# saiprasadbarke/robustmvd

Hardware: AMD Instinct MI355X
Metric: depth-maps/sec at 768x1152x4srcx256planes; warp+aggregate HBM GB/s vs roofline (higher is better)
Workload: dtype f32; 1 GPU; mvsnet (Path B) forward 768x1152, 4 source views, 256 planes, batch 1 per step (BASELINE.json configs[2]); the regulariser's two layers with 32 input channels (conv0, conv4): every fp32 operand as two range-scaled fp16 terms on fp16 MFMA, fp32 accumulation (at least as close to a float64 convolution as the fp32 matrix instruction over 1e-42..1e30: tests/test_hip_f16.py), the other nine layers and ; parallelism=1 independent replica(s), frames round-robin, no collectives

## Files before the change

### include/mvd.h

```cpp
#ifndef MVD_H_
#define MVD_H_

#include <stddef.h>

#ifdef __cplusplus
extern "C" {
#endif

#define MVD_VERSION 100
#define MVD_MAX_VIEWS 32

typedef void* mvd_stream_t;

typedef enum {
    MVD_OK = 0,
    MVD_ERR_INVALID_ARG = 1,
    MVD_ERR_WORKSPACE = 2,
    MVD_ERR_LAUNCH = 3,
    MVD_ERR_NO_DEVICE = 4
} mvd_status;

#define MVD_LAYOUT_NCDHW 0
#define MVD_LAYOUT_NDHWC 1
#define MVD_GRID_EXACT 0x100
#define MVD_FEAT_NHWC_BORDER 0x200

#define MVD_LAYOUT_NCHW 0
#define MVD_LAYOUT_NHWC 1
#define MVD_LAYOUT_NHWC_BORDER 2

int mvd_version(void);
const char* mvd_last_error(void);


size_t mvd_sweep_corr_workspace_bytes(int N, int C, int h, int w, int hs, int ws, int V);
int mvd_sweep_corr_f32(const float* feat_key, const float* const* feat_src, const float* K_key,
                       const float* const* K_src, const float* const* T_src2key, const float* invdepths,
                       int invdepth_batched, int N, int C, int h, int w, int hs, int ws, int S, int V,
                       float* const* corr_out, float* const* mask_out, void* workspace, size_t workspace_bytes,
                       mvd_stream_t stream);

#define MVD_INVDEPTH_SHARED 0
#define MVD_INVDEPTH_BATCHED 1
#define MVD_INVDEPTH_PER_PIXEL 2
int mvd_sweep_corr_ex_f32(const float* feat_key, const float* const* feat_src, const float* K_key,
                          const float* const* K_src, const float* const* T_src2key, const float* invdepths,
                          int invdepth_mode, float corr_scale, int N, int C, int h, int w, int hs, int ws, int S, int V,
                          float* const* corr_out, float* const* mask_out, void* workspace, size_t workspace_bytes,
                          mvd_stream_t stream);
int mvd_sweep_corr_nhwc_f32(const float* feat_key, const float* const* feat_src, const float* K_key, const float* const* K_src,
                            const float* const* T_src2key, const float* invdepths, int invdepth_mode, float corr_scale, int N, int C,
                            int h, int w, int hs, int ws, int S, int V, float* const* corr_out, float* const* mask_out,
                            int out_pixel_stride, float* corr_absmax, mvd_stream_t stream);

int mvd_sweep_warp_f32(const float* const* feat_src, const float* K_key, const float* const* K_src,
                       const float* const* T_src2key, const float* invdepths, int invdepth_mode, int normalize_after, int N,
                       int C, int h, int w, int hs, int ws, int S, int V, float* const* warped_out, float* const* mask_out,
                       mvd_stream_t stream);

int mvd_fuse_views_f32(const float* const* corr, const float* const* mask, const float* const* score, int N, int S,
                       int h, int w, int V, float* fused, float* fused_mask, mvd_stream_t stream);
int mvd_fuse_views_nhwc_f32(const float* const* corr, const float* const* mask, const float* const* score, int N, int S, int h,
                            int w, int V, int in_pixel_stride, float* fused, float* fused_mask, int out_pixel_stride,
                            float* fused_absmax, mvd_stream_t stream);


size_t mvd_warp_variance_workspace_bytes(int B, int C, int h, int w, int V);
int mvd_warp_variance_f32(const float* key_feat, const float* const* src_feat, const float* const* src_proj,
                          const float* key_proj_inv, const float* depth_values, int B, int C, int D, int h, int w,
                          int V, float* var_out, int out_layout, void* workspace, size_t workspace_bytes,
                          mvd_stream_t stream);
int mvd_warp_variance_absmax_f32(const float* key_feat, const float* const* src_feat, const float* const* src_proj,
                                 const float* key_proj_inv, const float* depth_values, int B, int C, int D, int h, int w,
                                 int V, float* var_out, float* absmax_out, int out_layout, void* workspace,
                                 size_t workspace_bytes, mvd_stream_t stream);

size_t mvd_warp_variance_f16_workspace_bytes(int B);
int mvd_warp_variance_f16(const void* key_feat, const void* const* src_feat, const float* const* src_proj,
                          const float* key_proj_inv, const float* depth_values, int B, int D, int h, int w, int V,
                          void* var_out, void* workspace, size_t workspace_bytes, mvd_stream_t stream);
int mvd_convert_f32_to_f16(const float* src, void* dst, long long n, mvd_stream_t stream);
int mvd_convert_f16_to_f32(const void* src, float* dst, long long n, mvd_stream_t stream);

int mvd_homo_warp_f32(const float* src_feat, const float* src_proj, const float* key_proj_inv,
                      const float* depth_values, int B, int C, int D, int h, int w, float* warped_out,
                      void* workspace, size_t workspace_bytes, mvd_stream_t stream);

#define MVD_CONV3D_STRIDE1 0
#define MVD_CONV3D_STRIDE2 1
#define MVD_DECONV3D_STRIDE2 2
size_t mvd_conv3d_packed_weight_floats(int Cin, int Cout);
int mvd_pack_conv3d_weights_f32(const float* w, int Cin, int Cout, int mode, float* packed, mvd_stream_t stream);
int mvd_conv3d_bn_relu_f32(const float* x, const float* packed_w, const float* scale, const float* shift,
                           const float* skip, float* y, int B, int Di, int hi, int wi, int Cin, int Cout, int mode,
                           int relu, mvd_stream_t stream);
int mvd_conv3d_bn_relu_absmax_f32(const float* x, const float* packed_w, const float* scale, const float* shift,
                                  const float* skip, float* y, float* absmax_out, int B, int Di, int hi, int wi, int Cin,
                                  int Cout, int mode, int relu, mvd_stream_t stream);

size_t mvd_conv3d_weight_grad_workspace_bytes(int B, int Di, int hi, int wi, int Cin, int Cout, int mode);
int mvd_conv3d_weight_grad_f32(const float* x, const float* gy, float* gw, int B, int Di, int hi, int wi, int Cin, int Cout,
                               int mode, void* workspace, size_t workspace_bytes, mvd_stream_t stream);

size_t mvd_conv3d_f16_packed_weight_bytes(int Cin, int Cout);
int mvd_pack_conv3d_weights_f16(const float* w, int Cin, int Cout, void* packed, mvd_stream_t stream);
int mvd_conv3d_bn_relu_f16in(const void* x, const void* packed_w, const float* scale, const float* shift, float* y, int B,
                             int D, int h, int w, int Cin, int Cout, int relu, mvd_stream_t stream);

size_t mvd_conv3d_split_packed_weight_bytes(int Cin, int Cout);
int mvd_pack_conv3d_weights_split(const float* w, int Cin, int Cout, void* packed, mvd_stream_t stream);
int mvd_conv3d_bn_relu_f32_split(const float* x, const float* x_absmax, const void* packed_w, const float* scale, const float* shift,
                                 float* y, int B, int D, int h, int w, int Cin, int Cout, int relu, mvd_stream_t stream);
int mvd_conv3d_bn_relu_absmax_f32_split(const float* x, const float* x_absmax, const void* packed_w, const float* scale, const float* shift,
                                        float* y, float* y_absmax, int B, int D, int h, int w, int Cin, int Cout, int relu,
                                        mvd_stream_t stream);
size_t mvd_conv3d_igemm_packed_weight_bytes(int Cin, int Cout, int mode);
int mvd_pack_conv3d_weights_igemm(const float* w, int Cin, int Cout, int mode, void* packed, mvd_stream_t stream);
size_t mvd_conv3d_igemm_workspace_bytes(int B, int Di, int Hi, int Wi, int Cin, int Cout, int mode);
int mvd_conv3d_bn_relu_igemm_f32(const float* x, const float* x_absmax, const void* packed_w, const float* scale, const float* shift,
                                 const float* skip, float* y, float* y_absmax, int B, int Di, int Hi, int Wi, int Cin, int Cout, int mode,
                                 int relu, void* workspace, size_t workspace_bytes, mvd_stream_t stream);
#define MVD_CONV2D 0
#define MVD_DECONV2D 1
#define MVD_CONV2D_IMAGE 2
size_t mvd_conv2d_split_packed_weight_bytes(int Cin_pad, int Cout, int KH, int KW, int stride, int mode);
int mvd_pack_conv2d_weights_split(const float* w, int Cin, int Cin_pad, int Cout, int KH, int KW, int stride, int mode, void* packed,
                                  mvd_stream_t stream);
size_t mvd_conv2d_split_workspace_bytes(int B, int Hi, int Wi, int Cin_pad, int Cout, int KH, int KW, int stride, int mode);
int mvd_conv2d_split_f32(const float* x, const float* x_absmax, const void* packed_w, const float* bias, float* y, float* y_absmax, int B,
                         int Hi, int Wi, int Cin_pad, int x_pixel_stride, int Cout, int y_pixel_stride, long long y_row_stride,
                         long long y_image_stride, long long y_channel_stride, int KH, int KW, int stride, int mode, int act, float slope,
                         void* workspace, size_t workspace_bytes, mvd_stream_t stream);
int mvd_upsample2x_nhwc_f32(const float* x, float* y, float* y_absmax, int B, int C, int h, int w, int y_pixel_stride, mvd_stream_t stream);
int mvd_absmax_f32(const float* x, long long n, float* absmax, mvd_stream_t stream);

size_t mvd_conv2d_packed_weight_floats(int Cin, int Cout, int ksize);
int mvd_pack_conv2d_weights_f32(const float* w, int Cin, int Cout, int ksize, float* packed, mvd_stream_t stream);
int mvd_conv2d_bn_relu_f32(const float* x, int in_layout, const float* packed_w, const float* scale, const float* shift,
                           float* y, int out_layout, int B, int hi, int wi, int Cin, int Cout, int ksize, int stride,
                           int relu, mvd_stream_t stream);
int mvd_conv2d_bn_relu_absmax_f32(const float* x, int in_layout, const float* packed_w, const float* scale, const float* shift,
                                  float* y, float* y_absmax, int out_layout, int B, int hi, int wi, int Cin, int Cout, int ksize,
                                  int stride, int relu, mvd_stream_t stream);

size_t mvd_conv2d_head_tile_count(int B, int H, int W);
int mvd_conv2d_head_f32(const float* image, const float* w0, const float* scale0, const float* shift0, const float* w1,
                        const float* scale1, const float* shift1, float* y, float* tile_absmax, int B, int H, int W,
                        mvd_stream_t stream);

int mvd_softmax_regress_f32(const float* cost, const float* depth_values, int B, int D, int h, int w,
                            float* depth_out, float* conf_out, mvd_stream_t stream);

int mvd_softmax_regress_stats_f32(const float* cost, const float* depth_values, int B, int D, int h, int w,
                                  float* depth_out, float* conf_out, float* stats_out, mvd_stream_t stream);
int mvd_softmax_regress_backward_f32(const float* cost, const float* depth_values, const float* depth, const float* stats,
                                     const float* g_depth, int B, int D, int h, int w, float* g_cost, mvd_stream_t stream);

int mvd_stream_fill_f32(float* dst, long long n, float value, mvd_stream_t stream);

int mvd_arm_kernel_timing(void* start_event, void* stop_event);

int mvd_bias_leaky_relu_f32(float* x, const float* bias, int N, int C, long long HW, float slope, mvd_stream_t stream);

#define MVD_REDUCE_VARIANCE 0
#define MVD_REDUCE_VARIANCE_KEYSQ 1
#define MVD_REDUCE_GROUPCORR 2
size_t mvd_sweep_reduce_workspace_bytes(int B, int C, int h, int w, int V);
int mvd_sweep_reduce_f32(const float* key_feat, const float* const* src_feat, const float* const* M, const float* depth,
                         int depth_per_pixel, float pix_offset, float scale_x, float scale_y, float bias, int mode, int groups,
                         int B, int C, int D, int h, int w, int V, float* const* out, void* workspace, size_t workspace_bytes,
                         mvd_stream_t stream);

int mvd_sweep_reduce_nhwc_f32(const float* key_feat, const float* const* src_feat, const float* const* M, const float* depth,
                              int depth_per_pixel, float pix_offset, float scale_x, float scale_y, float bias, int mode, int B, int C,
                              int D, int h, int w, int V, float* out, mvd_stream_t stream);

int mvd_softmax_regress_pp_f32(const float* cost, const float* depth_hypos, int B, int D, int h, int w, float* depth_out,
                               float* conf_out, mvd_stream_t stream);

int mvd_sweep_groupcorr_nhwc_f32(const float* key_feat, const float* const* src_feat, const float* const* M, const float* depth,
                                 int depth_per_pixel, float pix_offset, float scale_x, float scale_y, float bias, float grid_clamp,
                                 int groups, int B, int C, int D, int h, int w, int V, float* const* out, mvd_stream_t stream);

int mvd_soft_argmin_f32(const float* score, const float* depth_start, int start_per_pixel, const float* depth_interval, float window,
                        int B, int D, int h, int w, float* depth_out, float* entropy_out, float* prob_map_out, mvd_stream_t stream);

int mvd_vis_fuse_f32(const float* const* x, const float* const* u, int B, int D, int h, int w, int C, int V, float* out,
                     mvd_stream_t stream);


size_t mvd_warp_variance_backward_workspace_bytes(int B);
int mvd_warp_variance_backward_f32(const float* key_feat, const float* const* src_feat, const float* const* src_proj,
                                   const float* key_proj_inv, const float* depth_values, const float* grad_var, int B, int C,
                                   int D, int h, int w, int V, float* grad_key, float* const* grad_src, void* workspace,
                                   size_t workspace_bytes, mvd_stream_t stream);

#define MVD_K3_GATHER_RADIUS 3
size_t mvd_warp_variance_backward_gather_workspace_bytes(int B, int C, int D, int h, int w, int V);
int mvd_warp_variance_backward_gather_f32(const float* key_feat, const float* const* src_feat, const float* const* src_proj,
                                          const float* key_proj_inv, const float* depth_values, const float* grad_var, int B, int C,
                                          int D, int h, int w, int V, float* grad_key, float* const* grad_src, int* fallback_count,
                                          void* workspace, size_t workspace_bytes, mvd_stream_t stream);

int mvd_sweep_corr_backward_f32(const float* feat_key, const float* const* feat_src, const float* K_key,
                                const float* const* K_src, const float* const* T_src2key, const float* invdepths,
                                int invdepth_mode, float corr_scale, const float* const* grad_corr, int N, int C, int h, int w,
                                int hs, int ws, int S, int V, float* grad_key, float* const* grad_src, mvd_stream_t stream);

int mvd_sweep_warp_backward_f32(const float* K_key, const float* const* K_src, const float* const* T_src2key, const float* invdepths,
                                int invdepth_mode, const float* const* grad_warped, int N, int C, int h, int w, int hs, int ws, int S,
                                int V, float* const* grad_src, mvd_stream_t stream);

size_t mvd_sweep_reduce_backward_workspace_bytes(int B, int C, int h, int w, int V);
int mvd_sweep_reduce_backward_f32(const float* key_feat, const float* const* src_feat, const float* const* M, const float* depth,
                                  int depth_per_pixel, float pix_offset, float scale_x, float scale_y, float bias, int mode,
                                  int groups, const float* const* grad_out, int B, int C, int D, int h, int w, int V, float* grad_key,
                                  float* const* grad_src, void* workspace, size_t workspace_bytes, mvd_stream_t stream);

int mvd_fuse_views_backward_f32(const float* const* corr, const float* const* mask, const float* const* score,
                                const float* grad_fused, int N, int S, int h, int w, int V, float* const* grad_corr,
                                float* const* grad_score, mvd_stream_t stream);

int mvd_resize_order1_f32(const float* src, float* dst, long long planes, int hi, int wi, int ho, int wo,
                          mvd_stream_t stream);

int mvd_dispnet_head_f32(const float* x, float* pred, float* ent, int N, long long HW, mvd_stream_t stream);

#define MVD_ALIGN_NONE 0
#define MVD_ALIGN_MEDIAN 1
#define MVD_ALIGN_LSQ 2
size_t mvd_depth_eval_workspace_bytes(int H, int W);

int mvd_depth_align_stats_f32(const float* gt, const float* pred, const float* uncertainty, const int* row, const int* col, int H,
                              int W, int h, int w, int mode, int sparse_pred, float* params, double* sums, void* workspace,
                              size_t workspace_bytes, mvd_stream_t stream);

int mvd_depth_score_f32(const float* gt, const float* pred, const float* uncertainty, const int* row, const int* col, int H, int W,
                        int h, int w, int mode, int sparse_pred, int clip, float clip_lo, float clip_hi, float thresh,
                        float thresh_plus_one, const float* params, void* result, float* pred_out, float* invdepth_out,
                        float* rel_ae_out, float* uncertainty_out, void* workspace, size_t workspace_bytes, mvd_stream_t stream);

int mvd_rank_keys_f32(const float* u, const float* u_min, const float* gt, const float* pred_aligned, int sparse_pred, long long n,
                      float* keys, mvd_stream_t stream);

int mvd_ranked_step_sums_f64(const float* ranked, long long n, const long long* count, double* step_sums, void* workspace,
                             size_t workspace_bytes, mvd_stream_t stream);

int mvd_geo_consistency_f32(const float* key_depth, const float* const* src_depth, const float* matrices, const float* uncertainty,
                            int V, int H, int W, float max_reproj_error, float max_rel_depth_diff, int min_consistent_views,
                            float max_uncertainty, unsigned* view_bits, float* fused, unsigned char* mask,
                            unsigned char* num_consistent, mvd_stream_t stream);

size_t mvd_compact_points_workspace_bytes(int H, int W);
int mvd_compact_points_f32(const unsigned char* mask, const float* depth, const float* image, const float* backproject, int H, int W,
                           float* xyz, float* rgb, long long* count, void* workspace, size_t workspace_bytes, mvd_stream_t stream);

#define MVD_CLOUD_MAX_THRESHOLDS 8
int mvd_cloud_cell_keys_f32(const float* points, long long n, double origin_x, double origin_y, double origin_z, double inv,
                            long long* keys, mvd_stream_t stream);

int mvd_cloud_grid_build_f32(const float* points, const long long* perm, long long n, float* records, mvd_stream_t stream);

int mvd_cloud_nearest_f32(const float* query_records, long long n, const float* target_records, const long long* target_keys,
                          long long m, double origin_x, double origin_y, double origin_z, double inv, float max_dist, float* dist,
                          int* index, mvd_stream_t stream);

size_t mvd_cloud_scores_workspace_bytes(long long n);
int mvd_cloud_scores_f32(const float* dist, const int* index, const float* points, long long n, const float* thresholds, int T,
                         void* result, void* workspace, size_t workspace_bytes, mvd_stream_t stream);

size_t mvd_voxel_reduce_workspace_bytes(long long n);
int mvd_voxel_reduce_f32(const long long* keys, const long long* perm, const float* points, const float* colors, long long n,
                         float* xyz, float* rgb, int* counts, long long* num_voxels, void* workspace, size_t workspace_bytes,
                         mvd_stream_t stream);

int mvd_nchw_to_nhwc_f32(const float* src, float* dst, int N, int C, long long HW, mvd_stream_t stream);
int mvd_nhwc_to_nchw_f32(const float* src, float* dst, int N, int C, long long HW, mvd_stream_t stream);

#ifdef __cplusplus
}
#endif
#endif
```

### robustmvd_amd/_lib.py

```python
import ctypes
import os

import torch

_HERE = os.path.dirname(os.path.abspath(__file__))
LIB_PATH = os.path.join(_HERE, "lib", "libmvd_hip.so")
EXP_LIB_PATH = os.path.join(_HERE, "lib_exp", "libmvd_hip_exp.so")

MVD_MAX_VIEWS = 32
LAYOUT_NCDHW = 0
LAYOUT_NDHWC = 1
GRID_EXACT = 0x100
FEAT_NHWC_BORDER = 0x200
CONV3D_STRIDE1 = 0
CONV2D, DECONV2D, CONV2D_IMAGE = 0, 1, 2
CONV3D_STRIDE2 = 1
DECONV3D_STRIDE2 = 2
LAYOUT_NCHW = 0
LAYOUT_NHWC = 1
LAYOUT_NHWC_BORDER = 2
INVDEPTH_SHARED, INVDEPTH_BATCHED, INVDEPTH_PER_PIXEL = 0, 1, 2
REDUCE_VARIANCE = 0
REDUCE_VARIANCE_KEYSQ = 1
REDUCE_GROUPCORR = 2
ALIGN_NONE, ALIGN_MEDIAN, ALIGN_LSQ = 0, 1, 2
K3_GATHER_RADIUS = 3

_c_float_p = ctypes.c_void_p
_pp = ctypes.POINTER(ctypes.c_void_p)
_i = ctypes.c_int
_sz = ctypes.c_size_t

SIGNATURES = {
    "mvd_version": (_i, []),
    "mvd_last_error": (ctypes.c_char_p, []),
    "mvd_sweep_corr_workspace_bytes": (_sz, [_i] * 7),
    "mvd_sweep_corr_f32": (_i, [_c_float_p, _pp, _c_float_p, _pp, _pp, _c_float_p, _i] + [_i] * 8
                           + [_pp, _pp, ctypes.c_void_p, _sz, ctypes.c_void_p]),
    "mvd_sweep_corr_ex_f32": (_i, [_c_float_p, _pp, _c_float_p, _pp, _pp, _c_float_p, _i, ctypes.c_float] + [_i] * 8
                              + [_pp, _pp, ctypes.c_void_p, _sz, ctypes.c_void_p]),
    "mvd_sweep_corr_nhwc_f32": (_i, [_c_float_p, _pp, _c_float_p, _pp, _pp, _c_float_p, _i, ctypes.c_float] + [_i] * 8
                                + [_pp, _pp, _i, _c_float_p, ctypes.c_void_p]),
    "mvd_fuse_views_nhwc_f32": (_i, [_pp, _pp, _pp] + [_i] * 6 + [_c_float_p, _c_float_p, _i, _c_float_p, ctypes.c_void_p]),
    "mvd_upsample2x_nhwc_f32": (_i, [_c_float_p, _c_float_p, _c_float_p] + [_i] * 5 + [ctypes.c_void_p]),
    "mvd_sweep_warp_f32": (_i, [_pp, _c_float_p, _pp, _pp, _c_float_p] + [_i] * 10 + [_pp, _pp, ctypes.c_void_p]),
    "mvd_fuse_views_f32": (_i, [_pp, _pp, _pp, _i, _i, _i, _i, _i, _c_float_p, _c_float_p, ctypes.c_void_p]),
    "mvd_warp_variance_workspace_bytes": (_sz, [_i] * 5),
    "mvd_warp_variance_f32": (_i, [_c_float_p, _pp, _pp, _c_float_p, _c_float_p] + [_i] * 6
                              + [_c_float_p, _i, ctypes.c_void_p, _sz, ctypes.c_void_p]),
    "mvd_warp_variance_absmax_f32": (_i, [_c_float_p, _pp, _pp, _c_float_p, _c_float_p] + [_i] * 6
                                     + [_c_float_p, _c_float_p, _i, ctypes.c_void_p, _sz, ctypes.c_void_p]),
    "mvd_absmax_f32": (_i, [_c_float_p, ctypes.c_longlong, _c_float_p, ctypes.c_void_p]),
    "mvd_warp_variance_f16_workspace_bytes": (_sz, [_i]),
    "mvd_warp_variance_f16": (_i, [ctypes.c_void_p, _pp, _pp, _c_float_p, _c_float_p] + [_i] * 5
                              + [ctypes.c_void_p, ctypes.c_void_p, _sz, ctypes.c_void_p]),
    "mvd_convert_f32_to_f16": (_i, [_c_float_p, ctypes.c_void_p, ctypes.c_longlong, ctypes.c_void_p]),
    "mvd_convert_f16_to_f32": (_i, [ctypes.c_void_p, _c_float_p, ctypes.c_longlong, ctypes.c_void_p]),
    "mvd_homo_warp_f32": (_i, [_c_float_p] * 4 + [_i] * 5 + [_c_float_p, ctypes.c_void_p, _sz, ctypes.c_void_p]),
    "mvd_conv3d_packed_weight_floats": (_sz, [_i, _i]),
    "mvd_pack_conv3d_weights_f32": (_i, [_c_float_p, _i, _i, _i, _c_float_p, ctypes.c_void_p]),
    "mvd_conv3d_bn_relu_f32": (_i, [_c_float_p] * 6 + [_i] * 8 + [ctypes.c_void_p]),
    "mvd_conv3d_bn_relu_absmax_f32": (_i, [_c_float_p] * 7 + [_i] * 8 + [ctypes.c_void_p]),
    "mvd_conv3d_weight_grad_workspace_bytes": (_sz, [_i] * 7),
    "mvd_conv3d_weight_grad_f32": (_i, [_c_float_p] * 3 + [_i] * 7 + [ctypes.c_void_p, _sz, ctypes.c_void_p]),
    "mvd_conv3d_f16_packed_weight_bytes": (_sz, [_i, _i]),
    "mvd_pack_conv3d_weights_f16": (_i, [_c_float_p, _i, _i, ctypes.c_void_p, ctypes.c_void_p]),
    "mvd_conv3d_bn_relu_f16in": (_i, [ctypes.c_void_p, ctypes.c_void_p, _c_float_p, _c_float_p, _c_float_p] + [_i] * 7
                                 + [ctypes.c_void_p]),
    "mvd_conv3d_split_packed_weight_bytes": (_sz, [_i, _i]),
    "mvd_conv3d_bn_relu_absmax_f32_split": (_i, [_c_float_p, _c_float_p, ctypes.c_void_p, _c_float_p, _c_float_p, _c_float_p, _c_float_p]
                                            + [_i] * 7 + [ctypes.c_void_p]),
    "mvd_conv3d_igemm_packed_weight_bytes": (_sz, [_i] * 3),
    "mvd_pack_conv3d_weights_igemm": (_i, [_c_float_p, _i, _i, _i, ctypes.c_void_p, ctypes.c_void_p]),
    "mvd_conv3d_igemm_workspace_bytes": (_sz, [_i] * 7),
    "mvd_conv3d_bn_relu_igemm_f32": (_i, [_c_float_p, _c_float_p, ctypes.c_void_p] + [_c_float_p] * 5 + [_i] * 8
                                     + [ctypes.c_void_p, ctypes.c_size_t, ctypes.c_void_p]),
    "mvd_conv2d_split_packed_weight_bytes": (_sz, [_i] * 6),
    "mvd_pack_conv2d_weights_split": (_i, [_c_float_p] + [_i] * 7 + [ctypes.c_void_p, ctypes.c_void_p]),
    "mvd_conv2d_split_workspace_bytes": (_sz, [_i] * 9),
    "mvd_conv2d_split_f32": (_i, [_c_float_p, _c_float_p, ctypes.c_void_p, _c_float_p, _c_float_p, _c_float_p] + [_i] * 7
                             + [ctypes.c_longlong] * 3 + [_i] * 5 + [ctypes.c_float, ctypes.c_void_p, ctypes.c_size_t, ctypes.c_void_p]),
    "mvd_pack_conv3d_weights_split": (_i, [_c_float_p, _i, _i, ctypes.c_void_p, ctypes.c_void_p]),
    "mvd_conv3d_bn_relu_f32_split": (_i, [_c_float_p, _c_float_p, ctypes.c_void_p, _c_float_p, _c_float_p, _c_float_p] + [_i] * 7
                                     + [ctypes.c_void_p]),
    "mvd_conv2d_packed_weight_floats": (_sz, [_i, _i, _i]),
    "mvd_pack_conv2d_weights_f32": (_i, [_c_float_p, _i, _i, _i, _c_float_p, ctypes.c_void_p]),
    "mvd_conv2d_bn_relu_f32": (_i, [_c_float_p, _i, _c_float_p, _c_float_p, _c_float_p, _c_float_p, _i] + [_i] * 8
                               + [ctypes.c_void_p]),
    "mvd_conv2d_head_tile_count": (_sz, [_i] * 3),
    "mvd_conv2d_head_f32": (_i, [_c_float_p] * 9 + [_i] * 3 + [ctypes.c_void_p]),
    "mvd_conv2d_bn_relu_absmax_f32": (_i, [_c_float_p, _i, _c_float_p, _c_float_p, _c_float_p, _c_float_p, _c_float_p, _i] + [_i] * 8
                                      + [ctypes.c_void_p]),
    "mvd_softmax_regress_f32": (_i, [_c_float_p, _c_float_p, _i, _i, _i, _i, _c_float_p, _c_float_p, ctypes.c_void_p]),
    "mvd_softmax_regress_stats_f32": (_i, [_c_float_p, _c_float_p, _i, _i, _i, _i, _c_float_p, _c_float_p, _c_float_p,
                                           ctypes.c_void_p]),
    "mvd_softmax_regress_backward_f32": (_i, [_c_float_p] * 5 + [_i] * 4 + [_c_float_p, ctypes.c_void_p]),
    "mvd_bias_leaky_relu_f32": (_i, [_c_float_p, _c_float_p, _i, _i, ctypes.c_longlong, ctypes.c_float, ctypes.c_void_p]),
    "mvd_dispnet_head_f32": (_i, [_c_float_p, _c_float_p, _c_float_p, _i, ctypes.c_longlong, ctypes.c_void_p]),
    "mvd_arm_kernel_timing": (_i, [ctypes.c_void_p, ctypes.c_void_p]),
    "mvd_stream_fill_f32": (_i, [_c_float_p, ctypes.c_longlong, ctypes.c_float, ctypes.c_void_p]),
    "mvd_warp_variance_backward_workspace_bytes": (_sz, [_i]),
    "mvd_warp_variance_backward_f32": (_i, [_c_float_p, _pp, _pp, _c_float_p, _c_float_p, _c_float_p] + [_i] * 6
                                       + [_c_float_p, _pp, ctypes.c_void_p, _sz, ctypes.c_void_p]),
    "mvd_warp_variance_backward_gather_workspace_bytes": (_sz, [_i] * 6),
    "mvd_warp_variance_backward_gather_f32": (_i, [_c_float_p, _pp, _pp, _c_float_p, _c_float_p, _c_float_p] + [_i] * 6
                                              + [_c_float_p, _pp, ctypes.c_void_p, ctypes.c_void_p, _sz, ctypes.c_void_p]),
    "mvd_sweep_corr_backward_f32": (_i, [_c_float_p, _pp, _c_float_p, _pp, _pp, _c_float_p, _i, ctypes.c_float, _pp] + [_i] * 8
                                    + [_c_float_p, _pp, ctypes.c_void_p]),
    "mvd_fuse_views_backward_f32": (_i, [_pp, _pp, _pp, _c_float_p] + [_i] * 5 + [_pp, _pp, ctypes.c_void_p]),
    "mvd_sweep_reduce_workspace_bytes": (_sz, [_i] * 5),
    "mvd_sweep_reduce_f32": (_i, [_c_float_p, _pp, _pp, _c_float_p, _i] + [ctypes.c_float] * 4 + [_i] * 8
                             + [_pp, ctypes.c_void_p, _sz, ctypes.c_void_p]),
    "mvd_sweep_reduce_nhwc_f32": (_i, [_c_float_p, _pp, _pp, _c_float_p, _i] + [ctypes.c_float] * 4 + [_i] * 7
                                  + [_c_float_p, ctypes.c_void_p]),
    "mvd_softmax_regress_pp_f32": (_i, [_c_float_p, _c_float_p, _i, _i, _i, _i, _c_float_p, _c_float_p, ctypes.c_void_p]),
    "mvd_sweep_groupcorr_nhwc_f32": (_i, [_c_float_p, _pp, _pp, _c_float_p, _i] + [ctypes.c_float] * 5 + [_i] * 7 + [_pp, ctypes.c_void_p]),
    "mvd_soft_argmin_f32": (_i, [_c_float_p, _c_float_p, _i, _c_float_p, ctypes.c_float] + [_i] * 4 + [_c_float_p] * 3 + [ctypes.c_void_p]),
    "mvd_vis_fuse_f32": (_i, [_pp, _pp] + [_i] * 6 + [_c_float_p, ctypes.c_void_p]),
    "mvd_sweep_reduce_backward_workspace_bytes": (_sz, [_i] * 5),
    "mvd_sweep_reduce_backward_f32": (_i, [_c_float_p, _pp, _pp, _c_float_p, _i] + [ctypes.c_float] * 4 + [_i, _i, _pp] + [_i] * 6
                                      + [_c_float_p, _pp, ctypes.c_void_p, _sz, ctypes.c_void_p]),
    "mvd_sweep_warp_backward_f32": (_i, [_c_float_p, _pp, _pp, _c_float_p, _i, _pp] + [_i] * 8 + [_pp, ctypes.c_void_p]),
    "mvd_resize_order1_f32": (_i, [_c_float_p, _c_float_p, ctypes.c_longlong, _i, _i, _i, _i, ctypes.c_void_p]),
    "mvd_nchw_to_nhwc_f32": (_i, [_c_float_p, _c_float_p, _i, _i, ctypes.c_longlong, ctypes.c_void_p]),
    "mvd_nhwc_to_nchw_f32": (_i, [_c_float_p, _c_float_p, _i, _i, ctypes.c_longlong, ctypes.c_void_p]),
    "mvd_depth_eval_workspace_bytes": (_sz, [_i, _i]),
    "mvd_depth_align_stats_f32": (_i, [_c_float_p] * 3 + [ctypes.c_void_p] * 2 + [_i] * 6 + [_c_float_p, ctypes.c_void_p,
                                                                                            ctypes.c_void_p, _sz, ctypes.c_void_p]),
    "mvd_depth_score_f32": (_i, [_c_float_p] * 3 + [ctypes.c_void_p] * 2 + [_i] * 7 + [ctypes.c_float] * 4
                            + [_c_float_p, ctypes.c_void_p] + [_c_float_p] * 4 + [ctypes.c_void_p, _sz, ctypes.c_void_p]),
    "mvd_rank_keys_f32": (_i, [_c_float_p] * 4 + [_i, ctypes.c_longlong, _c_float_p, ctypes.c_void_p]),
    "mvd_ranked_step_sums_f64": (_i, [_c_float_p, ctypes.c_longlong, ctypes.c_void_p, ctypes.c_void_p, ctypes.c_void_p, _sz,
                                      ctypes.c_void_p]),
    "mvd_geo_consistency_f32": (_i, [_c_float_p, _pp, _c_float_p, _c_float_p, _i, _i, _i, ctypes.c_float, ctypes.c_float, _i,
                                     ctypes.c_float] + [ctypes.c_void_p] * 5),
    "mvd_compact_points_workspace_bytes": (_sz, [_i, _i]),
    "mvd_compact_points_f32": (_i, [ctypes.c_void_p] + [_c_float_p] * 3 + [_i, _i, _c_float_p, _c_float_p, ctypes.c_void_p,
                                                                          ctypes.c_void_p, _sz, ctypes.c_void_p]),
    "mvd_cloud_cell_keys_f32": (_i, [_c_float_p, ctypes.c_longlong] + [ctypes.c_double] * 4 + [ctypes.c_void_p] * 2),
    "mvd_cloud_grid_build_f32": (_i, [_c_float_p, ctypes.c_void_p, ctypes.c_longlong, _c_float_p, ctypes.c_void_p]),
    "mvd_cloud_nearest_f32": (_i, [_c_float_p, ctypes.c_longlong, _c_float_p, ctypes.c_void_p, ctypes.c_longlong]
                              + [ctypes.c_double] * 4 + [ctypes.c_float, _c_float_p, ctypes.c_void_p, ctypes.c_void_p]),
    "mvd_cloud_scores_workspace_bytes": (_sz, [ctypes.c_longlong]),
    "mvd_cloud_scores_f32": (_i, [_c_float_p, ctypes.c_void_p, _c_float_p, ctypes.c_longlong, _c_float_p, _i, ctypes.c_void_p,
                                  ctypes.c_void_p, _sz, ctypes.c_void_p]),
    "mvd_voxel_reduce_workspace_bytes": (_sz, [ctypes.c_longlong]),
    "mvd_voxel_reduce_f32": (_i, [ctypes.c_void_p] * 2 + [_c_float_p] * 2 + [ctypes.c_longlong, _c_float_p, _c_float_p]
                             + [ctypes.c_void_p] * 3 + [_sz, ctypes.c_void_p]),
}
MVD_CLOUD_MAX_THRESHOLDS = 8

PRODUCT_ONLY = ("mvd_sweep_reduce_backward_workspace_bytes", "mvd_sweep_reduce_backward_f32")

_lib = None
_override = None


def _bind(path, skip=()):
    lib = ctypes.CDLL(path)
    for name, (res, args) in SIGNATURES.items():
        if name in skip:
            continue
        fn = getattr(lib, name)
        fn.restype = res
        fn.argtypes = args
    return lib


def load():
    global _lib
    if _override is not None:
        return _override
    if _lib is not None:
        return _lib
    if not os.path.exists(LIB_PATH):
        raise RuntimeError(
            f"{LIB_PATH} not found: the HIP engine is not built. Run `python -c 'import __graft_entry__ as g; "
            "g.build()'` or `make -C robustmvd_amd/csrc`. There is no CPU fallback for this path.")
    _lib = _bind(LIB_PATH)
    return _lib


class use_experiments_library:

    def __init__(self, path=None):
        self.path = path or EXP_LIB_PATH

    def __enter__(self):
        global _override
        if not os.path.exists(self.path):
            raise RuntimeError(f"{self.path} not found: run `make -C robustmvd_amd/csrc exp`")
        self._prev = _override
        _override = _bind(self.path, skip=PRODUCT_ONLY)
        return _override

    def __exit__(self, *exc):
        global _override
        _override = self._prev
        return False


def check(rc, what):
    if rc != 0:
        msg = load().mvd_last_error().decode(errors="replace")
        raise RuntimeError(f"{what} failed (status {rc}): {msg}")


def stream_of(t):
    return ctypes.c_void_p(torch.cuda.current_stream(t.device).cuda_stream)


def raw_stream(device):
    return torch._C._cuda_getCurrentRawStream(device.index)


def ptr(t):
    return ctypes.c_void_p(t.data_ptr()) if t is not None else ctypes.c_void_p(0)


def ptr_array(tensors):
    arr = (ctypes.c_void_p * len(tensors))(*[t.data_ptr() for t in tensors])
    return ctypes.cast(arr, _pp), arr


def as_dtype(dtype, convert, t, name, shape=None, device=None):
    if not isinstance(t, torch.Tensor):
        raise ValueError(f"{name}: expected a torch.Tensor, got {type(t).__name__}")
    if not t.is_cuda:
        raise ValueError(f"{name}: tensor is on {t.device}; the HIP engine needs a cuda (ROCm) device tensor")
    if device is not None and t.device != device:
        raise ValueError(f"{name}: on {t.device}, expected {device}")
    if t.dtype != dtype:
        if not convert:
            raise ValueError(f"{name}: dtype {t.dtype}, expected {dtype}")
        t = t.to(dtype)
    if shape is not None and t.shape != tuple(shape):
        raise ValueError(f"{name}: shape {tuple(t.shape)}, expected {tuple(shape)}")
    return t.contiguous()


def as_f32(t, name, shape=None, device=None):
    return as_dtype(torch.float32, True, t, name, shape, device)


def as_f16(t, name, shape=None, device=None):
    return as_dtype(torch.float16, False, t, name, shape, device)
```

### robustmvd_amd/blocks.py

```python
import numpy as np
import torch
import torch.nn as nn
import torch.nn.functional as F

from . import _lib as L
from . import ops
from .utils import to_torch

homo_warp = ops.homo_warp


def compute_sampling_invdepths(min_depth, max_depth, num_samples, sampling_type="linear_invdepth"):
    def col(v):
        if isinstance(v, (float, int, np.floating)):
            v = torch.tensor([float(v)])
        return to_torch(v).float()[..., None]

    lo, hi = col(min_depth), col(max_depth)
    steps = torch.arange(0, num_samples, dtype=lo.dtype, device=lo.device)[None]
    if sampling_type == "linear_invdepth":
        return 1 / hi + steps * (1 / lo - 1 / hi) / (num_samples - 1)
    if sampling_type == "linear_depth":
        return (1 / (lo + steps * (hi - lo) / (num_samples - 1))).flip(1)
    raise ValueError(f"sampling_type {sampling_type!r}")


class PlanesweepCorrelation(nn.Module):

    def __init__(self, warp_only=False, normalize="dim", differentiable=False):
        super().__init__()
        self.warp_only = bool(warp_only)
        self.differentiable = bool(differentiable)
        allowed = ("dim", "before", "after", True, False) if warp_only else ("dim", "before", True, False)
        if normalize not in allowed:
            raise ValueError(f"normalize={normalize!r}: expected one of {allowed}")
        self.normalize = normalize
        self._invdepth_cache = {}

    def warm(self, num_sampling_points, min_depth, max_depth, sampling_type, device):
        ckey = (num_sampling_points, float(min_depth), float(max_depth), sampling_type, str(device))
        if ckey not in self._invdepth_cache:
            self._invdepth_cache[ckey] = compute_sampling_invdepths(min_depth, max_depth, num_sampling_points,
                                                                    sampling_type).to(device)
        return self._invdepth_cache[ckey]

    def forward(self, feat_key, intrinsics_key, feat_sources, source_to_key_transforms, intrinsics_sources=None,
                num_sampling_points=None, min_depth=None, max_depth=None, sampling_invdepths=None,
                sampling_type="linear_invdepth"):
        args = (feat_key, intrinsics_key, feat_sources, source_to_key_transforms, intrinsics_sources, num_sampling_points,
                min_depth, max_depth, sampling_invdepths, sampling_type)
        if self.warp_only:
            if ops.needs_grad(feat_sources):
                if not self.differentiable:
                    raise ValueError("PlanesweepCorrelation(warp_only=True): a source feature map requires grad; construct the "
                                     "block with differentiable=True for the engine's backward, or detach the features")
                return self._forward(ops.sweep_warp_autograd, *args)
            with torch.no_grad():
                return self._forward(ops.sweep_warp, *args)
        if ops.needs_grad(feat_key, feat_sources):
            return self._forward(ops.sweep_corr_autograd, *args)
        with torch.no_grad():
            return self._forward(ops.sweep_corr, *args)

    def _forward(self, sweep, feat_key, intrinsics_key, feat_sources, source_to_key_transforms, intrinsics_sources,
                 num_sampling_points, min_depth, max_depth, sampling_invdepths, sampling_type):
        if intrinsics_sources is None:
            intrinsics_sources = [intrinsics_key] * len(feat_sources)
        if not (len(feat_sources) == len(source_to_key_transforms) == len(intrinsics_sources)):
            raise ValueError("feat_sources, source_to_key_transforms and intrinsics_sources differ in length")
        if min_depth is not None and max_depth is not None:
            if sampling_invdepths is not None or num_sampling_points is None or sampling_type is None:
                raise ValueError("give either (num_sampling_points, min_depth, max_depth) or sampling_invdepths")
            scalars = all(isinstance(v, (float, int, np.floating)) for v in (min_depth, max_depth))
            ckey = (num_sampling_points, float(min_depth), float(max_depth), sampling_type, str(feat_key.device)) if scalars else None
            if ckey is not None and ckey in self._invdepth_cache:
                sampling_invdepths = self._invdepth_cache[ckey]
            else:
                sampling_invdepths = compute_sampling_invdepths(min_depth, max_depth, num_sampling_points, sampling_type)
                if ckey is not None:
                    sampling_invdepths = self._invdepth_cache[ckey] = sampling_invdepths.to(feat_key.device)
        elif num_sampling_points is not None or min_depth is not None or max_depth is not None or sampling_invdepths is None:
            raise ValueError("give either (num_sampling_points, min_depth, max_depth) or sampling_invdepths")
        inv = sampling_invdepths.to(feat_key.device)
        if inv.dim() < 2 or inv.dim() > 4:
            raise ValueError("sampling_invdepths must be (N, S), (N, S, H) or (N, S, H, W)")
        while inv.dim() < 4:
            inv = inv.unsqueeze(-1)
        inv_out = inv
        if inv.shape[2] == 1 and inv.shape[3] == 1:
            inv = inv.reshape(inv.shape[0], inv.shape[1])
        else:
            inv = inv.expand(feat_key.shape[0], inv.shape[1], feat_key.shape[2], feat_key.shape[3]).contiguous()
        if self.warp_only:
            srcs = list(feat_sources)
            if self.normalize == "before":
                srcs = [f / (torch.linalg.norm(f, dim=1, keepdim=True) + 1e-9) for f in srcs]
            after = self.normalize is True or self.normalize == "after"
            warped, masks = [None] * len(srcs), [None] * len(srcs)
            groups = {}
            for i, f in enumerate(srcs):
                groups.setdefault(tuple(f.shape[-2:]), []).append(i)
            for idxs in groups.values():
                wv, mv = sweep([srcs[i] for i in idxs], intrinsics_key, [intrinsics_sources[i] for i in idxs],
                                        [source_to_key_transforms[i] for i in idxs], inv, feat_key.shape[-2:], after)
                for i, wi, mi in zip(idxs, wv, mv):
                    warped[i], masks[i] = wi, mi
            return warped, masks, inv_out
        corr_scale = None
        if self.normalize != "dim":
            corr_scale = 1.0
            if self.normalize:
                nrm = lambda x: x / (torch.linalg.norm(x, dim=1, keepdim=True) + 1e-9)
                feat_key, feat_sources = nrm(feat_key), [nrm(f) for f in feat_sources]
        corrs = [None] * len(feat_sources)
        masks = [None] * len(feat_sources)
        groups = {}
        for i, f in enumerate(feat_sources):
            groups.setdefault(tuple(f.shape[-2:]), []).append(i)
        for idxs in groups.values():
            c, m = sweep(feat_key, [feat_sources[i] for i in idxs], intrinsics_key,
                         [intrinsics_sources[i] for i in idxs], [source_to_key_transforms[i] for i in idxs], inv, corr_scale)
            for i, ci, mi in zip(idxs, c, m):
                corrs[i], masks[i] = ci, mi
        return corrs, masks, inv_out


class LearnedFusion(nn.Module):
    def __init__(self):
        super().__init__()
        self.corr_to_view_weight = nn.Sequential(
            nn.Conv2d(256, 128, kernel_size=3, stride=1, padding=1, bias=True),
            nn.ReLU(inplace=True),
            nn.Conv2d(128, 1, kernel_size=1, stride=1, padding=0, bias=True),
        )

    def forward(self, corrs, masks):
        if len(corrs) == 1:
            return corrs[0], masks[0]
        n = corrs[0].shape[0]
        scores = self.corr_to_view_weight(torch.cat(list(corrs), 0))
        scores = list(torch.split(scores, n, 0))
        if ops.needs_grad(corrs, scores):
            return ops.fuse_views_autograd(corrs, masks, scores)
        return ops.fuse_views(corrs, masks, scores)


def depth_regression(p, depth_values):
    return torch.sum(p * depth_values.view(*depth_values.shape, 1, 1), 1)


class ConvBnReLU(nn.Module):
    def __init__(self, cin, cout, kernel_size=3, stride=1, pad=1):
        super().__init__()
        self.conv = nn.Conv2d(cin, cout, kernel_size, stride=stride, padding=pad, bias=False)
        self.bn = nn.BatchNorm2d(cout)

    def forward(self, x):
        return F.relu(self.bn(self.conv(x)), inplace=True)


def fold_bn(bn):
    scale = bn.weight / torch.sqrt(bn.running_var + bn.eps)
    return scale.detach().contiguous(), (bn.bias - bn.running_mean * scale).detach().contiguous()


class FeatureNetWeights:
    __slots__ = ("layers", "split", "head")

    def __init__(self):
        self.layers, self.split, self.head = [], [], ()

    def __getitem__(self, i):
        return self.layers[i]


class FeatureNet(nn.Module):

    SPEC = [(3, 8, 3, 1, 1), (8, 8, 3, 1, 1), (8, 16, 5, 2, 2), (16, 16, 3, 1, 1), (16, 16, 3, 1, 1),
            (16, 32, 5, 2, 2), (32, 32, 3, 1, 1)]

    def __init__(self, split_layers=True):
        super().__init__()
        self.inplanes = 32
        self.split_layers = bool(split_layers)
        self.fused_head = True
        for i, s in enumerate(self.SPEC):
            setattr(self, f"conv{i}", ConvBnReLU(*s))
        self.feature = nn.Conv2d(32, 32, 3, 1, 1)
        self._packed = None
        self._packed_key = None

    def _prepare(self):
        key = tuple((p.data_ptr(), p._version) for p in list(self.parameters()) + list(self.buffers()))
        if self._packed is not None and self._packed_key == key:
            return self._packed
        if self.training:
            raise RuntimeError("FeatureNet HIP path folds BatchNorm running statistics: call .eval() first")
        pk = FeatureNetWeights()
        for i, (cin, cout, k, stride, _) in enumerate(self.SPEC):
            m = getattr(self, f"conv{i}")
            w, _, _, _ = ops.pack_conv2d_weights(m.conv.weight.detach())
            pk.layers.append((w, cin, cout, k, stride, *fold_bn(m.bn), True))
        w, _, _, _ = ops.pack_conv2d_weights(self.feature.weight.detach())
        pk.layers.append((w, 32, 32, 3, 1, torch.ones(32, device=w.device), self.feature.bias.detach().contiguous(), False))
        if self.split_layers:
            for i in range(2, 8):
                conv = getattr(self, f"conv{i}").conv if i < 7 else self.feature
                _, _, _, _, stride, scale, shift, relu = pk.layers[i]
                pk.split.append((ops.pack_conv2d_weights_split(conv.weight.detach() * scale.view(-1, 1, 1, 1), shift, stride=stride), relu))
            for i in range(2):
                _, _, _, _, _, scale, shift, _ = pk.layers[i]
                pk.head += (getattr(self, f"conv{i}").conv.weight.detach().permute(2, 3, 1, 0).contiguous(), scale, shift)
        self._packed, self._packed_key = pk, key
        return pk

    @ops.inference_only
    def forward_layout(self, x, out_layout, return_absmax=False):
        pk = self._prepare()
        if not self.split_layers:
            for i, (w, cin, cout, k, stride, scale, shift, relu) in enumerate(pk.layers):
                x = ops.conv2d_bn_relu(x, w, cin, cout, k, stride, scale, shift, relu=relu,
                                       out_layout=out_layout if i == len(pk.layers) - 1 else L.LAYOUT_NHWC)
            return (x, ops.absmax(x)) if return_absmax else x
        slots = torch.zeros(8, dtype=torch.float32, device=x.device)
        if self.fused_head:
            x, a_in = ops.conv2d_head(x, *pk.head, return_absmax=True)
        else:
            for w, cin, cout, k, stride, scale, shift, relu in pk.layers[:2]:
                x = ops.conv2d_bn_relu(x, w, cin, cout, k, stride, scale, shift, relu=relu)
            a_in = ops.absmax(x)
        for j, (wts, relu) in enumerate(pk.split):
            last = j == len(pk.split) - 1
            if not last:
                x = ops.conv2d_split(x, a_in, wts, act=2 if relu else 0, out_absmax=slots[j:j + 1])
                a_in = slots[j:j + 1]
            elif out_layout == L.LAYOUT_NCHW:
                x = ops.conv2d_split(x, a_in, wts, act=0, planar_out=True)
                if return_absmax:
                    slots[7:8] = ops.absmax(x)
            elif out_layout == L.LAYOUT_NHWC_BORDER:
                B, h, w_, _ = x.shape
                buf = torch.zeros((B, h + 3, w_ + 3, wts.cout), dtype=torch.float32, device=x.device)
                ops.conv2d_split(x, a_in, wts, act=0, out=buf[:, 1:h + 1, 1:w_ + 1, :], out_absmax=slots[7:8])
                x = buf
            else:
                x = ops.conv2d_split(x, a_in, wts, act=0, out_absmax=slots[7:8])
        if return_absmax:
            return x, slots[7:8]
        return x

    def forward(self, x):
        return self.forward_layout(x, L.LAYOUT_NCHW)

    def forward_autograd(self, x):
        x = self.conv1(self.conv0(x))
        x = self.conv4(self.conv3(self.conv2(x)))
        return self.feature(self.conv6(self.conv5(x)))


class ConvBnReLU3D(nn.Module):
    def __init__(self, cin, cout, kernel_size=3, stride=1, pad=1):
        super().__init__()
        self.conv = nn.Conv3d(cin, cout, kernel_size, stride=stride, padding=pad, bias=False)
        self.bn = nn.BatchNorm3d(cout)

    def forward(self, x):
        return F.relu(self.bn(self.conv(x)), inplace=True)


def _deconv_block(cin, cout):
    return nn.Sequential(nn.ConvTranspose3d(cin, cout, kernel_size=3, padding=1, output_padding=1, stride=2, bias=False),
                         nn.BatchNorm3d(cout), nn.ReLU(inplace=True))


class CostRegNet(nn.Module):

    LAYERS = [("conv0", 32, 8, 1), ("conv1", 8, 16, 2), ("conv2", 16, 16, 1), ("conv3", 16, 32, 2), ("conv4", 32, 32, 1),
              ("conv5", 32, 64, 2), ("conv6", 64, 64, 1)]
    UPS = [("conv7", 64, 32), ("conv9", 32, 16), ("conv11", 16, 8)]

    def __init__(self, conv0_split=True):
        super().__init__()
        self.conv0_split = bool(conv0_split)
        for name, cin, cout, stride in self.LAYERS:
            setattr(self, name, ConvBnReLU3D(cin, cout, stride=stride))
        for name, cin, cout in self.UPS:
            setattr(self, name, _deconv_block(cin, cout))
        self.prob = nn.Conv3d(8, 1, 3, stride=1, padding=1)
        self._packed = None
        self._packed_key = None

    def _prepare(self):
        key = tuple((p.data_ptr(), p._version) for p in list(self.parameters()) + list(self.buffers()))
        if self._packed is not None and self._packed_key == key:
            return self._packed
        if self.training:
            raise RuntimeError("CostRegNet HIP path folds BatchNorm running statistics: call .eval() first")
        pk = {}
        for name, cin, cout, stride in self.LAYERS:
            m = getattr(self, name)
            mode = L.CONV3D_STRIDE1 if stride == 1 else L.CONV3D_STRIDE2
            w, _, _ = ops.pack_conv3d_weights(m.conv.weight.detach(), mode)
            pk[name] = (w, cin, cout, *fold_bn(m.bn), mode)
        for name, cin, cout in self.UPS:
            m = getattr(self, name)
            w, _, _ = ops.pack_conv3d_weights(m[0].weight.detach(), L.DECONV3D_STRIDE2)
            pk[name] = (w, cin, cout, *fold_bn(m[1]), L.DECONV3D_STRIDE2)
        w, _, _ = ops.pack_conv3d_weights(self.prob.weight.detach(), L.CONV3D_STRIDE1)
        pk["prob"] = (w, 8, 1, torch.ones(1, device=w.device), self.prob.bias.detach().contiguous(), L.CONV3D_STRIDE1)
        pk["conv0_f16"] = ops.pack_conv3d_weights_f16(self.conv0.conv.weight.detach())
        if self.conv0_split:
            pk["conv0_split"] = ops.pack_conv3d_weights_split(self.conv0.conv.weight.detach())
            sc0, sh0 = pk["conv0"][3], pk["conv0"][4]
            pk["conv0_bound"] = ((self.conv0.conv.weight.detach().abs().sum(dim=(1, 2, 3, 4)) * sc0.abs()).contiguous(), sh0.abs().contiguous())
            for name, _, _, stride in self.LAYERS:
                if name != "conv0":
                    pk[name + "_igemm"] = ops.pack_conv3d_weights_igemm(getattr(self, name).conv.weight.detach(),
                                                                        L.CONV3D_STRIDE1 if stride == 1 else L.CONV3D_STRIDE2)
        self._packed, self._packed_key = pk, key
        return pk

    @ops.inference_only
    def forward_channels_last(self, x, x_absmax=None):
        if x.shape[1] % 8 or x.shape[2] % 8 or x.shape[3] % 8:
            raise ValueError(f"CostRegNet needs D,h,w divisible by 8, got {tuple(x.shape[1:4])}")
        pk = self._prepare()

        def layer(name, t, relu=True, skip=None):
            w, cin, cout, scale, shift, mode = pk[name]
            return ops.conv3d_bn_relu(t, w, cin, cout, scale, shift, mode, relu=relu, skip=skip)

        if x.dtype == torch.float16:
            _, _, _, scale0, shift0, _ = pk["conv0"]
            conv0 = ops.conv3d_bn_relu_f16in(x, pk["conv0_f16"], scale0, shift0, relu=True)
            a0 = None
        elif self.conv0_split:
            _, _, _, scale0, shift0, _ = pk["conv0"]
            if x_absmax is None:
                x_absmax = ops.absmax(x)
            conv0 = ops.conv3d_bn_relu_split(x, pk["conv0_split"], scale0, shift0, relu=True, x_absmax=x_absmax)
            gain0, off0 = pk["conv0_bound"]
            a0 = (gain0 * x_absmax + off0).amax().reshape(1)
        else:
            conv0 = layer("conv0", x)
        if self.conv0_split:
            slots = torch.zeros(8, dtype=torch.float32, device=x.device)
            nslot = [0]

            def ig(name, t, a, want_absmax=True):
                _, cin, cout, sc, sh, mode = pk[name]
                out_a = None
                if want_absmax:
                    out_a = slots[nslot[0]:nslot[0] + 1]
                    nslot[0] += 1
                return ops.conv3d_bn_relu_igemm(t, a, pk[name + "_igemm"], cin, cout, sc, sh, mode, relu=True, return_absmax=want_absmax,
                                                out_absmax=out_a)

            if a0 is None:
                a0 = ops.absmax(conv0)
            t, a = ig("conv1", conv0, a0)
            conv2, a = ig("conv2", t, a)
            t, a = ig("conv3", conv2, a)
            conv4, a = ig("conv4", t, a)
            t, a = ig("conv5", conv4, a)
            y = ig("conv6", t, a, want_absmax=False)
        else:
            conv2 = layer("conv2", layer("conv1", conv0))
            conv4 = layer("conv4", layer("conv3", conv2))
            y = layer("conv6", layer("conv5", conv4))
        y = layer("conv7", y, skip=conv4)
        del conv4
        y = layer("conv9", y, skip=conv2)
        del conv2
        y = layer("conv11", y, skip=conv0)
        del conv0
        return layer("prob", y, relu=False).squeeze(-1)

    @ops.inference_only
    def forward(self, x):
        return self.forward_channels_last(ops.to_channels_last_3d(x)).unsqueeze(1)

    def forward_autograd(self, x):
        conv0 = self.conv0(x)
        conv2 = self.conv2(self.conv1(conv0))
        conv4 = self.conv4(self.conv3(conv2))
        x = self.conv6(self.conv5(conv4))
        x = conv4 + self.conv7(x)
        x = conv2 + self.conv9(x)
        x = conv0 + self.conv11(x)
        return self.prob(x)

    def forward_autograd_engine(self, x):
        if x.dim() != 5 or x.shape[1] % 8 or x.shape[2] % 8 or x.shape[3] % 8:
            raise ValueError(f"CostRegNet needs (B,D,h,w,32) with D,h,w divisible by 8, got {tuple(x.shape)}")

        def layer(name, t):
            m = getattr(self, name)
            stride = m.conv.stride[0]
            y = ops.conv3d_autograd(t, m.conv.weight, L.CONV3D_STRIDE1 if stride == 1 else L.CONV3D_STRIDE2)
            return F.relu(_batch_norm_channels_last(m.bn, y), inplace=True)

        def up(name, t):
            m = getattr(self, name)
            y = ops.conv3d_autograd(t, m[0].weight, L.DECONV3D_STRIDE2)
            return F.relu(_batch_norm_channels_last(m[1], y), inplace=True)

        conv0 = layer("conv0", x)
        conv2 = layer("conv2", layer("conv1", conv0))
        conv4 = layer("conv4", layer("conv3", conv2))
        x = layer("conv6", layer("conv5", conv4))
        x = conv4 + up("conv7", x)
        x = conv2 + up("conv9", x)
        x = conv0 + up("conv11", x)
        return (ops.conv3d_autograd(x, self.prob.weight, L.CONV3D_STRIDE1) + self.prob.bias).squeeze(-1)


def _batch_norm_channels_last(bn, y):
    factor = 0.0 if bn.momentum is None else bn.momentum
    if bn.training and bn.track_running_stats and bn.num_batches_tracked is not None:
        bn.num_batches_tracked.add_(1)
        if bn.momentum is None:
            factor = 1.0 / float(bn.num_batches_tracked)
    batch_stats = bn.training or (bn.running_mean is None and bn.running_var is None)
    keep = not bn.training or bn.track_running_stats
    out = F.batch_norm(y.reshape(-1, y.shape[-1]), bn.running_mean if keep else None, bn.running_var if keep else None,
                       bn.weight, bn.bias, batch_stats, factor, bn.eps)
    return out.view(y.shape)


class _ConvLeaky(nn.Sequential):

    def forward(self, x):
        c = self[0]
        if torch.is_grad_enabled() or not x.is_cuda or c.bias is None:
            return super().forward(x)
        if isinstance(c, nn.ConvTranspose2d):
            y = F.conv_transpose2d(x, c.weight, None, c.stride, c.padding, c.output_padding, c.groups, c.dilation)
        else:
            y = F.conv2d(x, c.weight, None, c.stride, c.padding, c.dilation, c.groups)
        if y.dtype != torch.float32 or not y.is_contiguous() or y.shape[0] * y.shape[1] > 65535:
            return F.leaky_relu(y + c.bias.to(y.dtype).view(1, -1, 1, 1), self[1].negative_slope, inplace=True)
        return ops.bias_leaky_relu_(y, c.bias, self[1].negative_slope)


def conv(cin, cout, kernel_size=3, stride=1):
    return _ConvLeaky(nn.Conv2d(cin, cout, kernel_size=kernel_size, stride=stride, padding=(kernel_size - 1) // 2, bias=True),
                      nn.LeakyReLU(0.2, inplace=True))


class ReLUAndSigmoid(nn.Module):

    def __init__(self, inplace=False, min=0.0, max=1.0):
        super().__init__()
        self.min, self.max, self.range = min, max, max - min

    def forward(self, x):
        return torch.cat([F.relu(x[:, :1]), torch.sigmoid(x[:, 1:] * (4 / self.range)) * self.range + self.min], 1)


class DispnetEncoder(nn.Module):
    def __init__(self):
        super().__init__()
        self.conv1 = conv(3, 64, kernel_size=7, stride=2)
        self.conv2 = conv(64, 128, kernel_size=5, stride=2)
        self.conv3 = conv(128, 256, kernel_size=3, stride=2)

    def forward(self, image):
        c1 = self.conv1(image)
        c2 = self.conv2(c1)
        c3 = self.conv3(c2)
        return {"conv1": c1, "conv2": c2, "conv3a": c3}, c3


class DispnetContextEncoder(nn.Module):
    def __init__(self):
        super().__init__()
        self.conv_redir = conv(256, 32, kernel_size=1, stride=1)

    def forward(self, conv3):
        return self.conv_redir(conv3)


class DispnetCostvolumeEncoder(nn.Module):
    def __init__(self):
        super().__init__()
        self.conv3_1 = conv(256 + 32, 256)
        self.conv4 = conv(256, 512, stride=2)
        self.conv4_1 = conv(512, 512)
        self.conv5 = conv(512, 512, stride=2)
        self.conv5_1 = conv(512, 512)
        self.conv6 = conv(512, 1024, stride=2)
        self.conv6_1 = conv(1024, 1024)

    def forward(self, corr, ctx):
        out = {"merged": torch.cat([ctx, corr], 1)}
        x = out["merged"]
        for name in ("conv3_1", "conv4", "conv4_1", "conv5", "conv5_1", "conv6", "conv6_1"):
            x = getattr(self, name)(x)
            out[name] = x
        return out, x


def _pred_block(cin):
    return nn.Sequential(nn.Conv2d(cin, 2, kernel_size=3, stride=1, padding=1, bias=True),
                         ReLUAndSigmoid(inplace=True, min=-10, max=10))


def _deconv(cin, cout):
    return _ConvLeaky(nn.ConvTranspose2d(cin, cout, kernel_size=4, stride=2, padding=1, bias=True),
                      nn.LeakyReLU(0.2, inplace=True))


def _iconv(cin, cout):
    return _ConvLeaky(nn.Conv2d(cin + 2, cout, kernel_size=3, stride=1, padding=1, bias=True),
                      nn.LeakyReLU(0.2, inplace=True))


class DispnetDecoder(nn.Module):

    SKIPS = ["conv5_1", "conv4_1", "conv3_1", "conv2", "conv1"]
    SKIP_CH = [512, 512, 256, 128, 64]

    def __init__(self):
        super().__init__()
        ch = 1024
        self.pred_0 = _pred_block(ch)
        for lvl, skip_ch in enumerate(self.SKIP_CH, start=1):
            nxt = ch // 2
            setattr(self, f"deconv_{lvl}", _deconv(ch, nxt))
            setattr(self, f"rfeat{lvl}", _iconv(nxt + skip_ch, nxt))
            setattr(self, f"pred_{lvl}", _pred_block(nxt))
            ch = nxt

    @staticmethod
    def _record(pred, preds, ent=None):
        mean, log_b = pred[:, 0:1], pred[:, 1:2]
        if ent is None:
            ent = torch.log(2 * torch.exp(log_b) + 1e-4) + 1
        preds.setdefault("invdepth_uncertainties_all", []).append(ent)
        preds.setdefault("invdepth_log_bs_all", []).append(log_b)
        preds.setdefault("invdepths_all", []).append(mean)
        preds["invdepth_uncertainty"], preds["invdepth_log_b"], preds["invdepth"] = ent, log_b, mean

    def _head(self, lvl, feat, preds):
        blk = getattr(self, f"pred_{lvl}")
# ... 17 lines not shown
```

### robustmvd_amd/csrc/conv2d_split.hip

```cpp
#include "mvd_common.h"
#include <algorithm>
#include <stdlib.h>

#ifndef C2_KO
#define C2_KO 0
#endif

namespace mvd {

typedef _Float16 c2h8 __attribute__((ext_vector_type(8)));
typedef float c2f4 __attribute__((ext_vector_type(4)));
typedef unsigned int c2u4 __attribute__((ext_vector_type(4)));
constexpr int C2_TH = 16, C2_TW = 16;

template <int KH, int KW, int S, int U8, bool IMG = false>
struct C2Geom {
    static constexpr int CC = 8 * U8;
    static constexpr int PB = 16;
    static constexpr int PH = (C2_TH - 1) * S + KH, PW = (C2_TW - 1) * S + KW;
    static constexpr int PWS = (PW + S - 1) / S;
    static constexpr int ROWB = S * S * PWS * PB;
    static constexpr int C8S = (PH * S * PWS * PB + 255) / 256 * 256;
    static constexpr int PLANE = U8 * C8S;
    static constexpr int UNITS = KH * KW * U8;
    static constexpr int STEPS = (UNITS + 3) / 4;
    static constexpr int ITEMS = PH * PW * U8;
    static constexpr int NIT = (ITEMS + 255) / 256;
    static_assert(2 * PLANE <= 80 * 1024, "patch exceeds half the LDS (two workgroups per CU)");
};
template <int KH, int KW, int S, int U8>
struct C2Geom<KH, KW, S, U8, true> {
    static_assert(KH == 7 && KW == 7 && S == 2 && U8 == 1, "image layer: 7 x 7, stride 2");
    static constexpr int CC = 8, PB = 8;
    static constexpr int PH = (C2_TH - 1) * S + KH, PW = (C2_TW - 1) * S + KW + 1;
    static constexpr int ROWB = S * PW * PB;
    static constexpr int PLANE = PH * PW * PB;
    static constexpr int STEPS = KH;
    static constexpr int ITEMS = PH * PW;
    static constexpr int NIT = (ITEMS + 255) / 256;
    static_assert(PW % 2 == 0, "16-byte aligned pixel pairs");
};

struct C2Params {
    const float* x;
    const float* xamax;
    const char* wpk;
    const float* eun;
    const float* bias;
    const float* scale;
    const float* skip;
    float* y;
    float* yamax;
    float* part;
    int B, Hi, Wi, xs, nchunks;
    int Di, Do, Dy, KD, SD, pad_d, nchunks_c, sub3d, Cr;
    int Ho, Wo;
    int Hy, Wy, ys;
    long long ys_row, ys_img, ycs;
    int oy_mul, ox_mul;
    int pad_y, pad_x;
    int Cout, ncp;
    int tiles_x, tiles_y, nblocks, ksplit, chunks_per_split;
    int ncls;
    long long cls_bytes;
    int act;
    float slope;
};

__global__ void c2_wscale_kernel(const float* __restrict__ w, float* __restrict__ eun, int Cin, int Cout, int taps, int transposed, int cpad) {
    __shared__ float red[256];
    const int c = blockIdx.x;
    float m = 0.f;
    if (c < Cout)
        for (int e = threadIdx.x; e < Cin * taps; e += 256) {
            const int ci = e / taps, t = e % taps;
            const float v = fabsf(transposed ? w[((size_t)ci * Cout + c) * taps + t] : w[((size_t)c * Cin + ci) * taps + t]);
            m = (v <= 3.4e38f && v > m) ? v : m;
        }
    red[threadIdx.x] = m;
    __syncthreads();
    for (int o = 128; o > 0; o >>= 1) {
        if (threadIdx.x < o) red[threadIdx.x] = fmaxf(red[threadIdx.x], red[threadIdx.x + o]);
        __syncthreads();
    }
    if (threadIdx.x == 0 && c < cpad) {
        const int ex = (int)((__float_as_uint(red[0]) >> 23) & 0xffu) - 127;
        const int k = red[0] > 0.f ? max(-100, min(100, ex - 10)) : 0;
        eun[c] = ldexpf(1.0f, k);
    }
}

__global__ void c2_pack_kernel(const float* __restrict__ w, const float* __restrict__ eun, _Float16* __restrict__ packed, int Cin, int Cout,
                               int KH, int KW, int U8, int nchunks, int ntiles, int steps, int transposed, long long total) {
    const long long e = (long long)blockIdx.x * 256 + threadIdx.x;
    if (e >= total) return;
    const int j = (int)(e & 7), lane = (int)((e >> 3) & 63), term = (int)((e >> 9) & 1);
    long long r = e >> 10;
    const int step = (int)(r % steps); r /= steps;
    const int chunk = (int)(r % nchunks); r /= nchunks;
    const int nt = (int)(r % ntiles);
    const int cls = (int)(r / ntiles);
    const int cout = nt * 16 + (lane & 15), unit = 4 * step + (lane >> 4);
    int tap = unit / U8, cin = chunk * 8 * U8 + 8 * (unit % U8) + j;
    if (transposed == 2) {
        const int kx = 2 * (lane >> 4) + j / 4;
        tap = kx < KW ? step * KW + kx : KH * KW;
        cin = j % 4;
    }
    float v = 0.f;
    if (tap < KH * KW && cin < Cin && cout < Cout) {
        const int ty = tap / KW, tx = tap % KW;
        if (transposed == 1) {
            const int a = cls >> 1, b = cls & 1, ky = 3 - a - 2 * ty, kx = 3 - b - 2 * tx;
            v = w[(((size_t)cin * Cout + cout) * 4 + ky) * 4 + kx];
        } else {
            v = w[(((size_t)cout * Cin + cin) * KH + ty) * KW + tx];
        }
        v = v / eun[cout];
    }
    const _Float16 hi = (_Float16)v;
    packed[e] = term == 0 ? hi : (_Float16)(v - (float)hi);
}

struct C2Chan {
    float mul[4], sc[4], bi[4];
};
__device__ __forceinline__ C2Chan c2_chan(const C2Params& p, int cb, float xsc_inv) {
    C2Chan k;
    const int c = p.sub3d ? cb % p.Cr : cb;
#pragma unroll
    for (int r = 0; r < 4; ++r) {
        const bool in = cb + r < p.Cout;
        k.mul[r] = in ? p.eun[cb + r] * xsc_inv : 0.f;
        k.sc[r] = (in && p.scale) ? p.scale[c + r] : 1.f;
        k.bi[r] = (in && p.bias) ? p.bias[c + r] : 0.f;
    }
    return k;
}
__device__ __forceinline__ size_t c2_out_offset(const C2Params& p, int b, int od, int oy, int ox, int cls, int cb) {
    int c = cb, zo = od, yo = oy * p.oy_mul + (cls >> 1), xo = ox * p.ox_mul + (cls & 1);
    if (p.sub3d) {
        const int k3 = cb / p.Cr;
        c = cb - k3 * p.Cr;
        zo = 2 * od + (k3 >> 2); yo = 2 * oy + ((k3 >> 1) & 1); xo = 2 * ox + (k3 & 1);
    }
    return ((size_t)b * p.Dy + zo) * p.ys_img + (size_t)yo * p.ys_row + (size_t)xo * p.ys + (size_t)c * p.ycs;
}
__device__ __forceinline__ size_t c2_row_step(const C2Params& p) { return (size_t)(p.sub3d ? 2 : p.oy_mul) * p.ys_row; }
__device__ __forceinline__ void c2_finish(const C2Params& p, size_t o, int cb, c2f4 a, const C2Chan& k, float& amax) {
    float r4[4];
#pragma unroll
    for (int r = 0; r < 4; ++r) {
        float v = 0.f;
        if (cb + r < p.Cout) {
            const float conv = a[r] * k.mul[r];
            v = p.scale ? fmaf(conv, k.sc[r], k.bi[r]) : conv + k.bi[r];
            if (p.act == 1) v = v > 0.f ? v : v * p.slope;
            else if (p.act == 2) v = fmaxf(v, 0.f);
            if (p.skip) v += p.skip[o + r * p.ycs];
            amax = fmaxf(amax, finite_abs_or_zero(v));
        }
        r4[r] = v;
    }
    if (cb + 3 < p.Cout && p.ycs == 1) {
        *reinterpret_cast<c2f4*>(p.y + o) = c2f4{r4[0], r4[1], r4[2], r4[3]};
    } else {
#pragma unroll
        for (int r = 0; r < 4; ++r)
            if (cb + r < p.Cout) p.y[o + r * p.ycs] = r4[r];
    }
}

template <int KH, int KW, int S, int U8, int WM, int NTW, bool NCHW3>
__global__ void __launch_bounds__(256, 2) conv2d_split_kernel(C2Params p) {
    const float amax_seen = absmax_seen(p.part ? nullptr : p.yamax);
    using G = C2Geom<KH, KW, S, U8, NCHW3>;
    constexpr int WN = 4 / WM, MTW = 16 / WM, STEPS = G::STEPS, PB = G::PB, PLANE = G::PLANE;
    extern __shared__ __attribute__((aligned(16))) char patch[];
    float* const wmax = reinterpret_cast<float*>(patch + 2 * PLANE);
    const int tid = threadIdx.x, lane = tid & 63, wv = tid >> 6;
    const int wm = wv / WN, wn = wv % WN;
    const int g = lane >> 4, px16 = lane & 15;

    int bx = blockIdx.x;
    const int nb = bx % p.nblocks; bx /= p.nblocks;
    const int ks = bx % p.ksplit; bx /= p.ksplit;
    const int cls = bx % p.ncls; bx /= p.ncls;
    const int tx = bx % p.tiles_x; bx /= p.tiles_x;
    const int ty = bx % p.tiles_y;
    const int b = bx / p.tiles_y;
    const int od = b % p.Do, bb = b / p.Do;
    const int ca = cls >> 1, cb2 = cls & 1;
    const int oy0 = ty * C2_TH, ox0 = tx * C2_TW;
    const int iy0 = oy0 * S - (p.pad_y - ca), ix0 = ox0 * S - (p.pad_x - cb2);

    float xsc, xsc_inv;
    {
        const unsigned mb = __builtin_amdgcn_readfirstlane((int)__float_as_uint(*p.xamax));
        const int ex = (int)((mb >> 23) & 0xffu) - 127;
        const int e = max(-125, min(125, ex - 14));
        xsc = __uint_as_float((unsigned)(127 - e) << 23);
        xsc_inv = __uint_as_float((unsigned)(127 + e) << 23);
    }
    const float one = 1.0f;
    auto split2 = [xsc, one](float a0, float a1, unsigned& hi, unsigned& lo) {
        unsigned hp, lp;
        float t0, t1;
        asm("v_fma_mixlo_f16 %0, %1, %2, 0 op_sel:[0,0,0] op_sel_hi:[0,0,0]" : "=v"(hp) : "v"(a0), "s"(xsc));
        asm("v_fma_mixhi_f16 %0, %1, %2, 0 op_sel:[0,0,0] op_sel_hi:[0,0,0]" : "+v"(hp) : "v"(a1), "s"(xsc));
        asm("v_fma_mix_f32 %0, %1, %2, -%3 op_sel:[0,0,0] op_sel_hi:[0,0,1]" : "=v"(t0) : "v"(a0), "s"(xsc), "v"(hp));
        asm("v_fma_mix_f32 %0, %1, %2, -%3 op_sel:[0,0,1] op_sel_hi:[0,0,1]" : "=v"(t1) : "v"(a1), "s"(xsc), "v"(hp));
        asm("v_fma_mixlo_f16 %0, %1, %2, 0 op_sel:[0,0,0] op_sel_hi:[0,0,0]" : "=v"(lp) : "v"(t0), "s"(one));
        asm("v_fma_mixhi_f16 %0, %1, %2, 0 op_sel:[0,0,0] op_sel_hi:[0,0,0]" : "+v"(lp) : "v"(t1), "s"(one));
        hi = hp;
        lo = lp;
    };

    long long goff[G::NIT];
    int loff[G::NIT];
#pragma unroll
    for (int k = 0; k < G::NIT; ++k) {
        const int it = tid + 256 * k;
        const int pix = it / U8, c8 = it % U8;
        const int py = pix / G::PW, pxx = pix % G::PW;
        const int iy = iy0 + py, ix = ix0 + pxx;
        const bool live = it < G::ITEMS;
        const bool inside = live && iy >= 0 && iy < p.Hi && ix >= 0 && ix < p.Wi;
        if constexpr (NCHW3) {
            goff[k] = inside ? ((long long)b * 3 * p.Hi + iy) * p.Wi + ix : -1;
            loff[k] = live ? pix * PB : -1;
        } else {
            goff[k] = inside ? ((long long)iy * p.Wi + ix) * p.xs + c8 * 8 : -1;
            loff[k] = live ? ((py * S + pxx % S) * G::PWS + pxx / S) * PB + c8 * G::C8S : -1;
        }
    }
    int tapoff[STEPS];
#pragma unroll
    for (int s = 0; s < STEPS; ++s) {
        if constexpr (NCHW3) {
            tapoff[s] = (s * G::PW + 2 * px16 + 2 * g) * PB + wm * MTW * G::ROWB;
        } else {
            int unit = 4 * s + g;
            if (unit >= G::UNITS) unit = 0;
            const int tap = unit / U8, c8 = unit % U8, ky = tap / KW, kx = tap % KW;
            tapoff[s] = ((ky * S + kx % S) * G::PWS + kx / S + px16) * PB + c8 * G::C8S + wm * MTW * G::ROWB;
        }
    }

    const int nt0 = nb * (WN * NTW) + wn * NTW;
    const size_t nt_stride = (size_t)p.nchunks * STEPS * 2048;
    const char* wlane = p.wpk + (size_t)cls * p.cls_bytes + (size_t)nt0 * nt_stride + lane * 16;

    c2f4 acc[MTW][NTW];
#pragma unroll
    for (int m = 0; m < MTW; ++m)
#pragma unroll
        for (int t = 0; t < NTW; ++t) acc[m][t] = c2f4{0, 0, 0, 0};

    const int c_begin = ks * p.chunks_per_split, c_end = min(p.nchunks, c_begin + p.chunks_per_split);

    c2h8 wh[NTW], wl[NTW];
    const char* wc = wlane + (size_t)c_begin * STEPS * 2048;
    const char* const wlast = wlane + ((size_t)max(c_end, c_begin + 1) * STEPS - 1) * 2048;
    if (c_begin < c_end) {
#pragma unroll
        for (int t = 0; t < NTW; ++t) {
            wh[t] = *reinterpret_cast<const c2h8*>(wc + t * nt_stride);
            wl[t] = *reinterpret_cast<const c2h8*>(wc + t * nt_stride + 1024);
        }
    }

    for (int chunk = c_begin; chunk < c_end; ++chunk) {
        if (!(C2_KO & 1) || chunk == c_begin) {
            c2f4 v0[G::NIT], v1[G::NIT];
            const int kd = chunk / p.nchunks_c, zi = od * p.SD - p.pad_d + kd;
            const bool zlive = zi >= 0 && zi < p.Di;
            const float* xim = p.x + ((size_t)bb * p.Di + (zlive ? zi : 0)) * p.Hi * p.Wi * p.xs + (size_t)(chunk - kd * p.nchunks_c) * G::CC;
#pragma unroll
            for (int k = 0; k < G::NIT; ++k) {
                v0[k] = c2f4{0, 0, 0, 0};
                v1[k] = c2f4{0, 0, 0, 0};
                if (goff[k] >= 0 && zlive) {
                    if constexpr (NCHW3) {
                        const size_t pl = (size_t)p.Hi * p.Wi;
                        v0[k][0] = p.x[goff[k]]; v0[k][1] = p.x[goff[k] + pl]; v0[k][2] = p.x[goff[k] + 2 * pl];
                    } else {
                        v0[k] = *reinterpret_cast<const c2f4*>(xim + goff[k]);
                        v1[k] = *reinterpret_cast<const c2f4*>(xim + goff[k] + 4);
                    }
                }
            }
            __syncthreads();
#pragma unroll
            for (int k = 0; k < G::NIT; ++k) {
                if (loff[k] < 0) continue;
                unsigned h0, h1, h2, h3, l0, l1, l2, l3;
                split2(v0[k][0], v0[k][1], h0, l0);
                split2(v0[k][2], v0[k][3], h1, l1);
                if constexpr (NCHW3) {
                    *reinterpret_cast<unsigned long long*>(patch + loff[k]) = (unsigned long long)h0 | ((unsigned long long)h1 << 32);
                    *reinterpret_cast<unsigned long long*>(patch + loff[k] + PLANE) = (unsigned long long)l0 | ((unsigned long long)l1 << 32);
                    continue;
                }
                split2(v1[k][0], v1[k][1], h2, l2);
                split2(v1[k][2], v1[k][3], h3, l3);
                *reinterpret_cast<c2u4*>(patch + loff[k]) = c2u4{h0, h1, h2, h3};
                *reinterpret_cast<c2u4*>(patch + loff[k] + PLANE) = c2u4{l0, l1, l2, l3};
            }
            __syncthreads();
        }

#pragma unroll
        for (int s = 0; s < STEPS; ++s) {
            c2h8 nh[NTW], nl[NTW];
            if (C2_KO & 4) {
#pragma unroll
                for (int t = 0; t < NTW; ++t) { nh[t] = wh[t]; nl[t] = wl[t]; }
            } else {
                const char* wn = wc + 2048;
                wn = wn > wlast ? wlast : wn;
#pragma unroll
                for (int t = 0; t < NTW; ++t) {
                    nh[t] = *reinterpret_cast<const c2h8*>(wn + t * nt_stride);
                    nl[t] = *reinterpret_cast<const c2h8*>(wn + t * nt_stride + 1024);
                }
                wc += 2048;
            }
            const char* a = patch + tapoff[s];
            c2h8 xh = *reinterpret_cast<const c2h8*>(a), xl = *reinterpret_cast<const c2h8*>(a + PLANE);
            c2h8 yh = xh, yl = xl;
            if (MTW > 1) {
                yh = *reinterpret_cast<const c2h8*>(a + G::ROWB);
                yl = *reinterpret_cast<const c2h8*>(a + G::ROWB + PLANE);
            }
#pragma unroll
            for (int m = 0; m < MTW; ++m) {
                const c2h8 ch = xh, cl = xl;
                xh = yh; xl = yl;
                if (m + 2 < MTW && !(C2_KO & 8)) {
                    yh = *reinterpret_cast<const c2h8*>(a + (m + 2) * G::ROWB);
                    yl = *reinterpret_cast<const c2h8*>(a + (m + 2) * G::ROWB + PLANE);
                }
#pragma unroll
                for (int t = 0; t < NTW; ++t) {
                    if (C2_KO & 2) {
                        acc[m][t][0] += (float)ch[0] * (float)wh[t][0] + (float)cl[1] * (float)wl[t][1];
                        continue;
                    }
                    acc[m][t] = __builtin_amdgcn_mfma_f32_16x16x32_f16(wh[t], ch, acc[m][t], 0, 0, 0);
                    acc[m][t] = __builtin_amdgcn_mfma_f32_16x16x32_f16(wl[t], ch, acc[m][t], 0, 0, 0);
                    acc[m][t] = __builtin_amdgcn_mfma_f32_16x16x32_f16(wh[t], cl, acc[m][t], 0, 0, 0);
                }
                __builtin_amdgcn_sched_barrier(0);
            }
#pragma unroll
            for (int t = 0; t < NTW; ++t) { wh[t] = nh[t]; wl[t] = nl[t]; }
        }
    }

    const int ox = ox0 + px16;
    float amax = 0.f;
#pragma unroll
    for (int t = 0; t < NTW; ++t) {
        const int cb = (nt0 + t) * 16 + 4 * g;
        if (p.part) {
            if (ox < p.Wo)
#pragma unroll
                for (int m = 0; m < MTW; ++m) {
                    const int oy = oy0 + wm * MTW + m;
                    if (oy >= p.Ho) continue;
                    const size_t pl = ((size_t)b * p.Ho + oy) * p.Wo + ox;
                    *reinterpret_cast<c2f4*>(p.part + (((size_t)cls * p.ksplit + ks) * p.B * p.Ho * p.Wo + pl) * p.ncp + cb) = acc[m][t];
                }
            continue;
        }
        if (cb >= p.Cout || ((C2_KO & 16) && p.B > 1000)) continue;
        const C2Chan kc = c2_chan(p, cb, xsc_inv);
        if (ox < p.Wo) {
            const size_t o0 = c2_out_offset(p, bb, od, oy0 + wm * MTW, ox, cls, cb), ostep = c2_row_step(p);
#pragma unroll
            for (int m = 0; m < MTW; ++m)
                if (oy0 + wm * MTW + m < p.Ho) c2_finish(p, o0 + m * ostep, cb, acc[m][t], kc, amax);
        }
    }
    if (p.yamax && !p.part) {
        for (int o = 32; o > 0; o >>= 1) amax = fmaxf(amax, __shfl_xor(amax, o));
        if (lane == 0) wmax[wv] = amax;
        __syncthreads();
        if (tid == 0) {
            amax = fmaxf(fmaxf(wmax[0], wmax[1]), fmaxf(wmax[2], wmax[3]));
            raise_absmax_seen(p.yamax, amax, amax_seen);
        }
    }
}

__global__ void __launch_bounds__(256) c2_reduce_kernel(C2Params p) {
    __shared__ float wmax[4];
    const int npix = p.B * p.Ho * p.Wo;
    const int c4n = (p.Cout + 3) / 4;
    const int cls = blockIdx.y;
    float xsc_inv;
    {
        const unsigned mb = __float_as_uint(*p.xamax);
        const int ex = (int)((mb >> 23) & 0xffu) - 127;
        const int e = max(-125, min(125, ex - 14));
        xsc_inv = __uint_as_float((unsigned)(127 + e) << 23);
    }
    float amax = 0.f;
    for (int i = blockIdx.x * 256 + threadIdx.x; i < npix * c4n; i += gridDim.x * 256) {
        const int pl = i / c4n;
        const int cb = (i - pl * c4n) * 4;
        const float* pp = p.part + ((size_t)cls * p.ksplit * npix + pl) * p.ncp + cb;
        const size_t kstr = (size_t)npix * p.ncp;
        c2f4 s = c2f4{0, 0, 0, 0};
        int ks = 0;
        for (; ks + 8 <= p.ksplit; ks += 8) {
            c2f4 v[8];
#pragma unroll
            for (int q = 0; q < 8; ++q) v[q] = *reinterpret_cast<const c2f4*>(pp + (size_t)(ks + q) * kstr);
#pragma unroll
            for (int q = 0; q < 8; ++q) s += v[q];
        }
        for (; ks + 2 <= p.ksplit; ks += 2) {
            const c2f4 v0 = *reinterpret_cast<const c2f4*>(pp + (size_t)ks * kstr), v1 = *reinterpret_cast<const c2f4*>(pp + (size_t)(ks + 1) * kstr);
            s += v0;
            s += v1;
        }
        const int row = pl / p.Wo, ox = pl - row * p.Wo, b = row / p.Ho, oy = row - b * p.Ho;
        const int bb = p.Do == 1 ? b : b / p.Do, od = b - bb * p.Do;
        c2_finish(p, c2_out_offset(p, bb, od, oy, ox, cls, cb), cb, s, c2_chan(p, cb, xsc_inv), amax);
    }
    if (p.yamax) {
        for (int o = 32; o > 0; o >>= 1) amax = fmaxf(amax, __shfl_xor(amax, o));
        if ((threadIdx.x & 63) == 0) wmax[threadIdx.x >> 6] = amax;
        __syncthreads();
        if (threadIdx.x == 0) {
            amax = fmaxf(fmaxf(wmax[0], wmax[1]), fmaxf(wmax[2], wmax[3]));
            raise_absmax(p.yamax, amax);
        }
    }
}

__global__ void __launch_bounds__(256) upsample2x_nhwc_kernel(const float* __restrict__ x, float* __restrict__ y, float* yamax, int B, int C, int h,
                                                              int w, int ys) {
    __shared__ float wmax[4];
    const long long n = (long long)B * 4 * h * w;
    float amax = 0.f;
    for (long long i = (long long)blockIdx.x * 256 + threadIdx.x; i < n; i += (long long)gridDim.x * 256) {
        const int ox = (int)(i % (2 * w)), oy = (int)((i / (2 * w)) % (2 * h)), b = (int)(i / (4LL * h * w));
        const float sy = fmaxf(0.5f * ((float)oy + 0.5f) - 0.5f, 0.f), sx = fmaxf(0.5f * ((float)ox + 0.5f) - 0.5f, 0.f);
        const int y0 = (int)sy, x0 = (int)sx;
        const int y1 = y0 + (y0 < h - 1 ? 1 : 0), x1 = x0 + (x0 < w - 1 ? 1 : 0);
        const float ly1 = sy - (float)y0, ly0 = 1.f - ly1, lx1 = sx - (float)x0, lx0 = 1.f - lx1;
        for (int c = 0; c < C; ++c) {
            const float* pl = x + ((size_t)b * C + c) * h * w;
            const float v = ly0 * (lx0 * pl[(size_t)y0 * w + x0] + lx1 * pl[(size_t)y0 * w + x1]) +
                            ly1 * (lx0 * pl[(size_t)y1 * w + x0] + lx1 * pl[(size_t)y1 * w + x1]);
            y[(size_t)i * ys + c] = v;
            amax = fmaxf(amax, finite_abs_or_zero(v));
        }
    }
    if (yamax) {
        for (int o = 32; o > 0; o >>= 1) amax = fmaxf(amax, __shfl_xor(amax, o));
        if ((threadIdx.x & 63) == 0) wmax[threadIdx.x >> 6] = amax;
        __syncthreads();
        if (threadIdx.x == 0) {
            amax = fmaxf(fmaxf(wmax[0], wmax[1]), fmaxf(wmax[2], wmax[3]));
            raise_absmax(yamax, amax);
        }
    }
}

__device__ __forceinline__ int c3_deconv_kidx(int a, int t) { return a == 0 ? (t == 0 ? 1 : -1) : (t == 0 ? 2 : 0); }

__global__ void c3_pack_kernel(const float* __restrict__ w, const float* __restrict__ eun, _Float16* __restrict__ packed, int Cin, int Cout,
                               int U8, int nchunks_c, int ntiles, int steps, int transposed, long long total) {
    const long long e = (long long)blockIdx.x * 256 + threadIdx.x;
    if (e >= total) return;
    const int KD = transposed ? 2 : 3, KP = transposed ? 2 : 3;
    const int j = (int)(e & 7), lane = (int)((e >> 3) & 63), term = (int)((e >> 9) & 1);
    long long r = e >> 10;
    const int step = (int)(r % steps); r /= steps;
    const int chunk = (int)(r % (KD * nchunks_c)); r /= KD * nchunks_c;
    const int nt = (int)r;
    const int kd = chunk / nchunks_c, cc = chunk % nchunks_c;
    const int ce = nt * 16 + (lane & 15), unit = 4 * step + (lane >> 4);
    const int tap = unit / U8, cin = cc * 8 * U8 + 8 * (unit % U8) + j;
    const int ncout = transposed ? 8 * Cout : Cout;
    float v = 0.f;
    if (tap < KP * KP && cin < Cin && ce < ncout) {
        const int ty = tap / KP, tx = tap % KP;
        if (transposed) {
            const int k3 = ce / Cout, c = ce % Cout;
            const int kz = c3_deconv_kidx(k3 >> 2, kd), ky = c3_deconv_kidx((k3 >> 1) & 1, ty), kx = c3_deconv_kidx(k3 & 1, tx);
            if (kz >= 0 && ky >= 0 && kx >= 0) v = w[((((size_t)cin * Cout + c) * 3 + kz) * 3 + ky) * 3 + kx];
        } else {
            v = w[((((size_t)ce * Cin + cin) * 3 + kd) * 3 + ty) * 3 + tx];
        }
        v = v / eun[ce];
    }
    const _Float16 hi = (_Float16)v;
    packed[e] = term == 0 ? hi : (_Float16)(v - (float)hi);
}

__global__ void c3_wscale_kernel(const float* __restrict__ w, float* __restrict__ eun, int Cin, int Cout, int transposed, int ncout, int cpad) {
    __shared__ float red[256];
    const int ce = blockIdx.x, c = ce % Cout;
    float m = 0.f;
    if (ce < ncout)
        for (int e = threadIdx.x; e < Cin * 27; e += 256) {
            const int ci = e / 27, t = e % 27;
            const float v = fabsf(transposed ? w[((size_t)ci * Cout + c) * 27 + t] : w[((size_t)c * Cin + ci) * 27 + t]);
            m = (v <= 3.4e38f && v > m) ? v : m;
        }
    red[threadIdx.x] = m;
    __syncthreads();
    for (int o = 128; o > 0; o >>= 1) {
        if (threadIdx.x < o) red[threadIdx.x] = fmaxf(red[threadIdx.x], red[threadIdx.x + o]);
        __syncthreads();
    }
    if (threadIdx.x == 0 && ce < cpad) {
        const int ex = (int)((__float_as_uint(red[0]) >> 23) & 0xffu) - 127;
        const int k = red[0] > 0.f ? max(-100, min(100, ex - 10)) : 0;
        eun[ce] = ldexpf(1.0f, k);
    }
}

struct C2Shape {
    int KH, KW, S, U8, steps;
    bool transposed, nchw3;
};

static bool c2_shape(int KH, int KW, int stride, int mode, int cin_pad, C2Shape* s) {
    s->transposed = mode == 1;
    s->nchw3 = mode == 2;
    s->KH = KH; s->KW = KW; s->S = stride;
    if (mode == 1) {
        if (KH != 4 || KW != 4 || stride != 2 || cin_pad % 32) return false;
        s->KH = s->KW = 2; s->S = 1; s->U8 = 4;
    } else if (mode == 2) {
        if (KH != 7 || KW != 7 || stride != 2 || cin_pad != 8) return false;
        s->U8 = 1;
        s->steps = 7;
        return true;
    } else if (KH == 1 && KW == 1 && stride == 1) {
        if (cin_pad % 32) return false;
        s->U8 = 4;
    } else if (KH == 3 && KW == 3 && stride == 1) {
        s->U8 = cin_pad % 32 == 0 ? 4 : 1;
    } else if ((KH == 3 && KW == 3 && stride == 2) || (KH == 5 && KW == 5 && stride == 2)) {
        s->U8 = 1;
    } else {
        return false;
    }
    if (cin_pad % (8 * s->U8)) return false;
    s->steps = (s->KH * s->KW * s->U8 + 3) / 4;
    return true;
}

static int c2_bn(int cout) {
    if (const char* e = exp_env("MVD_C2_BN")) {
        const int v = atoi(e);
        if (v == 16 || v == 32 || v == 64 || v == 128) return v;
    }
    return cout > 64 ? 128 : cout > 32 ? 64 : cout > 16 ? 32 : 16;
}
static int c2_ntiles(int cout) { return (cout + c2_bn(cout) - 1) / c2_bn(cout) * (c2_bn(cout) / 16); }
static size_t c2_frag_bytes(const C2Shape& s, int cin_pad, int cout) {
    const size_t nchunks = (size_t)cin_pad / (8 * s.U8);
    return (s.transposed ? 4 : 1) * (size_t)c2_ntiles(cout) * nchunks * s.steps * 2048;
}
static int c2_cpad(int cout) { return (cout + 127) / 128 * 128; }

struct C2Plan {
    int Ho, Wo, tiles_x, tiles_y, bn, nblocks, ncp, ncls, nchunks, ksplit;
    long long tiles;
    size_t part_bytes;
};
static C2Plan c2_plan(const C2Shape& s, int B, int Hi, int Wi, int cin_pad, int cout, int KH, int KW, int stride) {
    C2Plan q{};
    if (s.transposed) { q.Ho = Hi; q.Wo = Wi; q.ncls = 4; }
    else { q.Ho = (Hi + 2 * (KH / 2) - KH) / stride + 1; q.Wo = (Wi + 2 * (KW / 2) - KW) / stride + 1; q.ncls = 1; }
    q.tiles_y = (q.Ho + C2_TH - 1) / C2_TH;
    q.tiles_x = (q.Wo + C2_TW - 1) / C2_TW;
    q.bn = c2_bn(cout);
    q.nblocks = (cout + q.bn - 1) / q.bn;
    q.ncp = q.nblocks * q.bn;
    q.nchunks = cin_pad / (8 * s.U8);
    q.tiles = (long long)q.tiles_x * q.tiles_y * B * q.nblocks * q.ncls;
    q.ksplit = 1;
    if (q.tiles < 128)
        while (q.tiles * q.ksplit < 320 && q.ksplit < 32 && q.nchunks / (q.ksplit * 2) >= 2) q.ksplit *= 2;
    if (const char* e = exp_env("MVD_C2_KSPLIT")) {
        const int v = atoi(e);
        if (v >= 1 && v <= 32 && (v & (v - 1)) == 0 && v <= q.nchunks) q.ksplit = v;
    }
    q.part_bytes = q.ksplit > 1 ? (size_t)q.ksplit * q.ncls * B * q.Ho * q.Wo * q.ncp * sizeof(float) : 0;
    return q;
}

template <int KH, int KW, int S, int U8, int WM, int NTW, bool NCHW3>
static int c2_launch(const C2Params& p, long long nblk, hipStream_t st) {
    using G = C2Geom<KH, KW, S, U8, NCHW3>;
    auto kern = conv2d_split_kernel<KH, KW, S, U8, WM, NTW, NCHW3>;
    constexpr int lds = 2 * G::PLANE + 16;
    static_assert(lds <= 80 * 1024, "two workgroups per CU");
    if (lds > 48 * 1024 && hipFuncSetAttribute((const void*)kern, hipFuncAttributeMaxDynamicSharedMemorySize, lds) != hipSuccess)
        return launch_status("conv2d_split: LDS attribute");
    hipLaunchKernelGGL(kern, dim3((unsigned)nblk), dim3(256), lds, st, p);
    return launch_status("conv2d_split");
}

template <int KH, int KW, int S, int U8, bool NCHW3>
static int c2_launch_bn(const C2Params& p, int bn, long long nblk, hipStream_t st) {
    switch (bn) {
        case 128: return c2_launch<KH, KW, S, U8, 1, 2, NCHW3>(p, nblk, st);
        case 64: return c2_launch<KH, KW, S, U8, 1, 1, NCHW3>(p, nblk, st);
        case 32: return c2_launch<KH, KW, S, U8, 2, 1, NCHW3>(p, nblk, st);
        case 16: return c2_launch<KH, KW, S, U8, 4, 1, NCHW3>(p, nblk, st);
    }
    return MVD_ERR_INVALID_ARG;
}

static int c2_dispatch(const C2Shape& s, const C2Params& p, int bn, long long nblk, hipStream_t st) {
    if (s.nchw3) return c2_launch_bn<7, 7, 2, 1, true>(p, bn, nblk, st);
    if (s.KH == 1) return c2_launch_bn<1, 1, 1, 4, false>(p, bn, nblk, st);
    if (s.KH == 2) return s.U8 == 4 ? c2_launch_bn<2, 2, 1, 4, false>(p, bn, nblk, st) : c2_launch_bn<2, 2, 1, 2, false>(p, bn, nblk, st);
    if (s.KH == 5) return c2_launch_bn<5, 5, 2, 1, false>(p, bn, nblk, st);
    if (s.S == 2) return c2_launch_bn<3, 3, 2, 1, false>(p, bn, nblk, st);
    if (s.U8 == 4) return c2_launch_bn<3, 3, 1, 4, false>(p, bn, nblk, st);
    return c2_launch_bn<3, 3, 1, 1, false>(p, bn, nblk, st);
}

}

extern "C" {

size_t mvd_conv2d_split_packed_weight_bytes(int Cin_pad, int Cout, int KH, int KW, int stride, int mode) {
    mvd::C2Shape s;
    if (Cin_pad <= 0 || Cout <= 0 || !mvd::c2_shape(KH, KW, stride, mode, Cin_pad, &s)) return 0;
    return mvd::c2_frag_bytes(s, Cin_pad, Cout) + (size_t)mvd::c2_cpad(Cout) * sizeof(float);
}

int mvd_pack_conv2d_weights_split(const float* w, int Cin, int Cin_pad, int Cout, int KH, int KW, int stride, int mode, void* packed,
                                  mvd_stream_t stream) {
    MVD_REQUIRE(w && packed, "pack_conv2d_weights_split: NULL argument");
    mvd::C2Shape s;
    MVD_REQUIRE(Cin > 0 && Cin <= Cin_pad && Cout > 0 && mvd::c2_shape(KH, KW, stride, mode, Cin_pad, &s),
                "pack_conv2d_weights_split: layer %dx%d stride %d mode %d with %d (padded %d) -> %d channels is not built", KH, KW, stride, mode,
                Cin, Cin_pad, Cout);
    hipStream_t st = (hipStream_t)stream;
    const size_t fb = mvd::c2_frag_bytes(s, Cin_pad, Cout);
    float* eun = reinterpret_cast<float*>(static_cast<char*>(packed) + fb);
    const int cpad = mvd::c2_cpad(Cout);
    hipLaunchKernelGGL(mvd::c2_wscale_kernel, dim3(cpad), dim3(256), 0, st, w, eun, Cin, Cout, KH * KW, s.transposed ? 1 : 0, cpad);
    const long long total = (long long)(fb / 2);
    hipLaunchKernelGGL(mvd::c2_pack_kernel, dim3((unsigned)((total + 255) / 256)), dim3(256), 0, st, w, eun, (_Float16*)packed, Cin, Cout, s.KH,
                       s.KW, s.U8, Cin_pad / (8 * s.U8), mvd::c2_ntiles(Cout), s.steps, s.transposed ? 1 : s.nchw3 ? 2 : 0, total);
    return mvd::launch_status("pack_conv2d_weights_split");
}

size_t mvd_conv2d_split_workspace_bytes(int B, int Hi, int Wi, int Cin_pad, int Cout, int KH, int KW, int stride, int mode) {
    mvd::C2Shape s;
    if (B <= 0 || Hi <= 0 || Wi <= 0 || Cin_pad <= 0 || Cout <= 0 || !mvd::c2_shape(KH, KW, stride, mode, Cin_pad, &s)) return 0;
    return mvd::c2_plan(s, B, Hi, Wi, Cin_pad, Cout, KH, KW, stride).part_bytes;
}

int mvd_conv2d_split_f32(const float* x, const float* x_absmax, const void* packed_w, const float* bias, float* y, float* y_absmax, int B,
                         int Hi, int Wi, int Cin_pad, int x_pixel_stride, int Cout, int y_pixel_stride, long long y_row_stride,
                         long long y_image_stride, long long y_channel_stride, int KH, int KW, int stride, int mode, int act, float slope,
                         void* workspace, size_t workspace_bytes, mvd_stream_t stream) {
    MVD_REQUIRE(x && x_absmax && packed_w && y, "conv2d_split: NULL argument");
    MVD_REQUIRE(B > 0 && Hi > 0 && Wi > 0, "conv2d_split: non-positive dimension");
    mvd::C2Shape s;
    MVD_REQUIRE(Cin_pad > 0 && Cout > 0 && mvd::c2_shape(KH, KW, stride, mode, Cin_pad, &s),
                "conv2d_split: layer %dx%d stride %d mode %d with %d -> %d channels is not built", KH, KW, stride, mode, Cin_pad, Cout);
    MVD_REQUIRE(mode == 2 || (x_pixel_stride >= Cin_pad && x_pixel_stride % 4 == 0), "conv2d_split: input pixel stride %d (channels %d)",
                x_pixel_stride, Cin_pad);
    if (y_channel_stride <= 0) y_channel_stride = 1;
    MVD_REQUIRE(y_channel_stride != 1 || y_pixel_stride >= Cout, "conv2d_split: output pixel stride %d below %d channels", y_pixel_stride, Cout);
    MVD_REQUIRE(y_pixel_stride >= 1 && y_row_stride >= 0 && y_image_stride >= 0, "conv2d_split: negative output stride");
    MVD_REQUIRE(act >= 0 && act <= 2, "conv2d_split: act=%d unknown", act);
    MVD_REQUIRE(mode == 2 || (((uintptr_t)x & 15) == 0 && ((uintptr_t)y & 15) == 0), "conv2d_split: x and y must be 16-byte aligned");
    hipStream_t st = (hipStream_t)stream;
    mvd::C2Params p{};
    p.x = x; p.xamax = x_absmax; p.bias = bias; p.y = y; p.yamax = y_absmax;
    p.B = B; p.Hi = Hi; p.Wi = Wi; p.xs = x_pixel_stride; p.nchunks = Cin_pad / (8 * s.U8);
    p.Di = p.Do = p.Dy = p.KD = p.SD = 1; p.pad_d = 0; p.nchunks_c = p.nchunks; p.sub3d = 0; p.Cr = Cout;
    p.Cout = Cout; p.ys = y_pixel_stride; p.act = act; p.slope = slope;
    const size_t fb = mvd::c2_frag_bytes(s, Cin_pad, Cout);
    p.eun = reinterpret_cast<const float*>(static_cast<const char*>(packed_w) + fb);
    const mvd::C2Plan q = mvd::c2_plan(s, B, Hi, Wi, Cin_pad, Cout, KH, KW, stride);
    p.Ho = q.Ho; p.Wo = q.Wo; p.ncls = q.ncls;
    if (s.transposed) {
        p.Hy = 2 * Hi; p.Wy = 2 * Wi; p.oy_mul = p.ox_mul = 2; p.pad_y = p.pad_x = 1;
    } else {
        p.Hy = p.Ho; p.Wy = p.Wo; p.oy_mul = p.ox_mul = 1; p.pad_y = KH / 2; p.pad_x = KW / 2;
    }
    MVD_REQUIRE(y_channel_stride != 1 || Cout < 4 || (y_pixel_stride % 4 == 0 && y_row_stride % 4 == 0 && y_image_stride % 4 == 0),
                "conv2d_split: channel-last output strides must be multiples of 4 floats");
    p.ycs = y_channel_stride;
    p.ys_row = y_row_stride > 0 ? y_row_stride : (long long)p.Wy * y_pixel_stride;
    p.ys_img = y_image_stride > 0 ? y_image_stride : (long long)p.Hy * p.ys_row;
    p.wpk = static_cast<const char*>(packed_w);
    p.cls_bytes = (long long)(fb / p.ncls);
    p.tiles_y = q.tiles_y; p.tiles_x = q.tiles_x;
    const int bn = q.bn;
    p.nblocks = q.nblocks;
    p.ncp = q.ncp;
    const long long tiles = q.tiles;
    int ksplit = q.ksplit;
    if (ksplit > 1 && (!workspace || workspace_bytes < q.part_bytes)) ksplit = 1;
    p.ksplit = ksplit;
    p.chunks_per_split = (p.nchunks + ksplit - 1) / ksplit;
    p.part = ksplit > 1 ? static_cast<float*>(workspace) : nullptr;
    const long long nblk = tiles * ksplit;
    MVD_REQUIRE(nblk <= 0x7fffffffLL, "conv2d_split: %lld workgroups exceed the grid limit", nblk);
    int rc = mvd::c2_dispatch(s, p, bn, nblk, st);
    if (rc != MVD_OK || ksplit == 1) return rc;
    const long long n = (long long)B * p.Ho * p.Wo * ((Cout + 3) / 4);
    MVD_REQUIRE(n < 0x7fffffffLL, "conv2d_split: split reduction over %lld outputs", n);
    hipLaunchKernelGGL(mvd::c2_reduce_kernel, dim3((unsigned)std::min<long long>((n + 255) / 256, 1024), (unsigned)p.ncls), dim3(256), 0, st, p);
    return mvd::launch_status("conv2d_split: reduce");
}

int mvd_upsample2x_nhwc_f32(const float* x, float* y, float* y_absmax, int B, int C, int h, int w, int y_pixel_stride, mvd_stream_t stream) {
    MVD_REQUIRE(x && y, "upsample2x_nhwc: NULL argument");
    MVD_REQUIRE(B > 0 && C > 0 && h > 0 && w > 0 && y_pixel_stride >= C, "upsample2x_nhwc: bad dimension");
    const long long n = (long long)B * 4 * h * w;
    hipLaunchKernelGGL(mvd::upsample2x_nhwc_kernel, dim3((unsigned)std::min<long long>((n + 255) / 256, 1024)), dim3(256), 0, (hipStream_t)stream, x, y,
                       y_absmax, B, C, h, w, y_pixel_stride);
    return mvd::launch_status("upsample2x_nhwc");
}

}

namespace mvd {
static bool c3_shape(int Cin, int Cout, int mode, C2Shape* s, int* ncout) {
    if (Cin <= 0 || Cin % 8 || Cout <= 0 || Cout % 4 || mode < 0 || mode > 2) return false;
    s->transposed = false; s->nchw3 = false;
    if (mode == MVD_DECONV3D_STRIDE2) {
        if (Cin % 16) return false;
        s->KH = s->KW = 2; s->S = 1; s->U8 = Cin % 32 == 0 ? 4 : 2;
        *ncout = 8 * Cout;
    } else {
        s->KH = s->KW = 3; s->S = mode == MVD_CONV3D_STRIDE2 ? 2 : 1;
        s->U8 = (s->S == 1 && Cin % 32 == 0) ? 4 : 1;
        *ncout = Cout;
    }
    s->steps = (s->KH * s->KW * s->U8 + 3) / 4;
    return true;
}
static size_t c3_frag_bytes(const C2Shape& s, int Cin, int ncout, int mode) {
    const size_t KD = mode == MVD_DECONV3D_STRIDE2 ? 2 : 3;
    return (size_t)c2_ntiles(ncout) * KD * (Cin / (8 * s.U8)) * s.steps * 2048;
}
}

extern "C" {

size_t mvd_conv3d_igemm_packed_weight_bytes(int Cin, int Cout, int mode) {
    mvd::C2Shape s;
    int ncout;
    if (!mvd::c3_shape(Cin, Cout, mode, &s, &ncout)) return 0;
    return mvd::c3_frag_bytes(s, Cin, ncout, mode) + (size_t)mvd::c2_cpad(ncout) * sizeof(float);
}

int mvd_pack_conv3d_weights_igemm(const float* w, int Cin, int Cout, int mode, void* packed, mvd_stream_t stream) {
    MVD_REQUIRE(w && packed, "pack_conv3d_weights_igemm: NULL argument");
    mvd::C2Shape s;
    int ncout;
    MVD_REQUIRE(mvd::c3_shape(Cin, Cout, mode, &s, &ncout), "pack_conv3d_weights_igemm: %d -> %d channels, mode %d is not built", Cin, Cout, mode);
    hipStream_t st = (hipStream_t)stream;
    const size_t fb = mvd::c3_frag_bytes(s, Cin, ncout, mode);
    float* eun = reinterpret_cast<float*>(static_cast<char*>(packed) + fb);
    const int cpad = mvd::c2_cpad(ncout), tr = mode == MVD_DECONV3D_STRIDE2 ? 1 : 0;
    hipLaunchKernelGGL(mvd::c3_wscale_kernel, dim3(cpad), dim3(256), 0, st, w, eun, Cin, Cout, tr, ncout, cpad);
    const long long total = (long long)(fb / 2);
    hipLaunchKernelGGL(mvd::c3_pack_kernel, dim3((unsigned)((total + 255) / 256)), dim3(256), 0, st, w, eun, (_Float16*)packed, Cin, Cout, s.U8,
                       Cin / (8 * s.U8), mvd::c2_ntiles(ncout), s.steps, tr, total);
    return mvd::launch_status("pack_conv3d_weights_igemm");
}

static mvd::C2Plan c3_plan(const mvd::C2Shape& s, int B, int Di, int Hi, int Wi, int Cin, int ncout, int mode, int* Do) {
    mvd::C2Plan q{};
    const int sd = mode == MVD_CONV3D_STRIDE2 ? 2 : 1;
    *Do = Di / sd; q.Ho = Hi / sd; q.Wo = Wi / sd; q.ncls = 1;
    q.tiles_y = (q.Ho + mvd::C2_TH - 1) / mvd::C2_TH;
    q.tiles_x = (q.Wo + mvd::C2_TW - 1) / mvd::C2_TW;
    q.bn = mvd::c2_bn(ncout);
    q.nblocks = (ncout + q.bn - 1) / q.bn;
    q.ncp = q.nblocks * q.bn;
    q.nchunks = (mode == MVD_DECONV3D_STRIDE2 ? 2 : 3) * (Cin / (8 * s.U8));
    q.tiles = (long long)q.tiles_x * q.tiles_y * B * *Do * q.nblocks;
    q.ksplit = 1;
    if (q.tiles < 128)
        while (q.tiles * q.ksplit < 320 && q.ksplit < 32 && q.nchunks / (q.ksplit * 2) >= 2) q.ksplit *= 2;
    q.part_bytes = q.ksplit > 1 ? (size_t)q.ksplit * B * *Do * q.Ho * q.Wo * q.ncp * sizeof(float) : 0;
    return q;
}

size_t mvd_conv3d_igemm_workspace_bytes(int B, int Di, int Hi, int Wi, int Cin, int Cout, int mode) {
    mvd::C2Shape s;
    int ncout, Do;
    if (B <= 0 || Di <= 0 || Hi <= 0 || Wi <= 0 || !mvd::c3_shape(Cin, Cout, mode, &s, &ncout)) return 0;
    return c3_plan(s, B, Di, Hi, Wi, Cin, ncout, mode, &Do).part_bytes;
}

int mvd_conv3d_bn_relu_igemm_f32(const float* x, const float* x_absmax, const void* packed_w, const float* scale, const float* shift,
                                 const float* skip, float* y, float* y_absmax, int B, int Di, int Hi, int Wi, int Cin, int Cout, int mode,
                                 int relu, void* workspace, size_t workspace_bytes, mvd_stream_t stream) {
    MVD_REQUIRE(x && x_absmax && packed_w && scale && shift && y, "conv3d_igemm: NULL argument");
    MVD_REQUIRE(B > 0 && Di > 0 && Hi > 0 && Wi > 0, "conv3d_igemm: non-positive dimension");
    mvd::C2Shape s;
    int ncout;
    MVD_REQUIRE(mvd::c3_shape(Cin, Cout, mode, &s, &ncout), "conv3d_igemm: %d -> %d channels, mode %d is not built", Cin, Cout, mode);
    MVD_REQUIRE(mode != MVD_CONV3D_STRIDE2 || (Di % 2 == 0 && Hi % 2 == 0 && Wi % 2 == 0), "conv3d_igemm stride 2: odd input dims %dx%dx%d", Di, Hi, Wi);
    MVD_REQUIRE((((uintptr_t)x | (uintptr_t)y | (uintptr_t)skip) & 15) == 0, "conv3d_igemm: x, y and skip must be 16-byte aligned");
    hipStream_t st = (hipStream_t)stream;
    int Do;
    const mvd::C2Plan q = c3_plan(s, B, Di, Hi, Wi, Cin, ncout, mode, &Do);
    const bool tr = mode == MVD_DECONV3D_STRIDE2;
    mvd::C2Params p{};
    p.x = x; p.xamax = x_absmax; p.bias = shift; p.scale = scale; p.skip = skip; p.y = y; p.yamax = y_absmax;
    p.wpk = static_cast<const char*>(packed_w);
    p.eun = reinterpret_cast<const float*>(p.wpk + mvd::c3_frag_bytes(s, Cin, ncout, mode));
    p.B = B * Do; p.Hi = Hi; p.Wi = Wi; p.xs = Cin; p.nchunks = q.nchunks;
    p.Di = Di; p.Do = Do; p.KD = tr ? 2 : 3; p.SD = mode == MVD_CONV3D_STRIDE2 ? 2 : 1; p.pad_d = tr ? 0 : 1; p.nchunks_c = Cin / (8 * s.U8);
    p.sub3d = tr ? 1 : 0; p.Cr = Cout; p.Dy = tr ? 2 * Di : Do;
    p.Ho = q.Ho; p.Wo = q.Wo; p.Hy = tr ? 2 * Hi : q.Ho; p.Wy = tr ? 2 * Wi : q.Wo;
    p.oy_mul = p.ox_mul = 1; p.pad_y = p.pad_x = tr ? 0 : 1;
    p.Cout = ncout; p.ncp = q.ncp; p.ys = Cout; p.ycs = 1;
    p.ys_row = (long long)p.Wy * Cout; p.ys_img = (long long)p.Hy * p.ys_row;
    p.tiles_x = q.tiles_x; p.tiles_y = q.tiles_y; p.nblocks = q.nblocks; p.ncls = 1; p.cls_bytes = 0;
    p.act = relu ? 2 : 0; p.slope = 0.f;
    int ksplit = q.ksplit;
    if (ksplit > 1 && (!workspace || workspace_bytes < q.part_bytes)) ksplit = 1;
    p.ksplit = ksplit;
    p.chunks_per_split = (p.nchunks + ksplit - 1) / ksplit;
    p.part = ksplit > 1 ? static_cast<float*>(workspace) : nullptr;
    const long long nblk = q.tiles * ksplit;
    MVD_REQUIRE(nblk <= 0x7fffffffLL, "conv3d_igemm: %lld workgroups exceed the grid limit", nblk);
    int rc = mvd::c2_dispatch(s, p, q.bn, nblk, st);
    if (rc != MVD_OK || ksplit == 1) return rc;
    const long long n = (long long)p.B * p.Ho * p.Wo * ((p.Cout + 3) / 4);
    MVD_REQUIRE(n < 0x7fffffffLL, "conv3d_igemm: split reduction over %lld outputs", n);
    hipLaunchKernelGGL(mvd::c2_reduce_kernel, dim3((unsigned)std::min<long long>((n + 255) / 256, 1024)), dim3(256), 0, st, p);
    return mvd::launch_status("conv3d_igemm: reduce");
}
}
```

### robustmvd_amd/csrc/resize.hip

```cpp
#include "mvd_common.h"

namespace mvd {

struct AxisTap {
    int i0, i1;
    double w0, w1;
};

__device__ __forceinline__ AxisTap axis_tap(int o, int n_in, int n_out) {
    AxisTap t;
    if (n_in <= 1) {
        t.i0 = t.i1 = 0; t.w0 = 1.0; t.w1 = 0.0;
        return t;
    }
    const double zoom = (double)n_in / (double)n_out;
    double c = ((double)o + 0.5) * zoom - 0.5;
    const double last = (double)(n_in - 1), sz2 = 2.0 * last;
    if (c < 0.0) c = -c;
    if (c > last) c = sz2 - c;
    const double st = floor(c);
    t.w1 = c - st;
    t.w0 = 1.0 - t.w1;
    t.i0 = (int)st;
    t.i1 = t.i0 + 1;
    if (t.i1 > n_in - 1) t.i1 = 2 * (n_in - 1) - t.i1;
    return t;
}

__global__ void __launch_bounds__(256) resize_order1_kernel(const float* __restrict__ src, float* __restrict__ dst, int hi, int wi,
                                                            int ho, int wo) {
    const int x = blockIdx.x * 256 + threadIdx.x;
    const int y = blockIdx.y;
    const size_t plane = blockIdx.z;
    if (x >= wo) return;
    const AxisTap ty = axis_tap(y, hi, ho), tx = axis_tap(x, wi, wo);
    const float* __restrict__ s = src + plane * (size_t)hi * wi;
    const double a00 = s[(size_t)ty.i0 * wi + tx.i0], a01 = s[(size_t)ty.i0 * wi + tx.i1];
    const double a10 = s[(size_t)ty.i1 * wi + tx.i0], a11 = s[(size_t)ty.i1 * wi + tx.i1];
    double t = (a00 * ty.w0) * tx.w0;
    t = t + (a01 * ty.w0) * tx.w1;
    t = t + (a10 * ty.w1) * tx.w0;
    t = t + (a11 * ty.w1) * tx.w1;
    dst[(plane * ho + y) * (size_t)wo + x] = (float)t;
}

}

extern "C" int mvd_resize_order1_f32(const float* src, float* dst, long long planes, int hi, int wi, int ho, int wo,
                                     mvd_stream_t stream) {
    MVD_REQUIRE(src && dst, "resize_order1: NULL argument");
    MVD_REQUIRE(planes > 0 && planes <= 65535 && hi > 0 && wi > 0, "resize_order1: bad dimensions (planes 1..65535)");
    MVD_REQUIRE(ho >= hi && wo >= wi && ho <= 65535,
                "resize_order1: only upscaling is built (%dx%d -> %dx%d): downscaling takes skimage's anti-aliasing filter", hi,
                wi, ho, wo);
    const dim3 grid((unsigned)((wo + 255) / 256), (unsigned)ho, (unsigned)planes);
    hipLaunchKernelGGL(mvd::resize_order1_kernel, grid, dim3(256), 0, (hipStream_t)stream, src, dst, hi, wi, ho, wo);
    return mvd::launch_status("resize_order1");
}
```

### robustmvd_amd/ops.py

```python
import functools
import itertools

import torch

from . import _lib as L


def _tensors(obj):
    if isinstance(obj, torch.Tensor):
        yield obj
    elif isinstance(obj, (list, tuple)):
        for o in obj:
            yield from _tensors(o)
    elif isinstance(obj, dict):
        for o in obj.values():
            yield from _tensors(o)


def inference_only(fn):
    @functools.wraps(fn)
    def wrapper(*args, **kwargs):
        if torch.is_grad_enabled():
            if any(t.requires_grad for t in _tensors((args, kwargs))):
                raise RuntimeError(f"{fn.__qualname__}: an input requires grad, but this HIP path is inference-only (no "
# ... 620 lines not shown
    return None if both[0, 0] == float("inf") else both


def _cloud_origin(origin, name="origin"):
    o = [float(v) for v in (origin.tolist() if hasattr(origin, "tolist") else origin)]
    if len(o) != 3 or not all(abs(v) < float("inf") for v in o):
        raise ValueError(f"{name} must be 3 finite numbers, got {o}")
    return o


def _check_cloud_indices(extent, origin, inv, what, edge):
    if extent is None:
        return
    lo = [(extent[0, a] - origin[a]) * inv for a in range(3)]
    hi = [(extent[1, a] - origin[a]) * inv for a in range(3)]
    if min(lo) < 0 or max(hi) >= CLOUD_INDEX_LIMIT:
        raise ValueError(f"{what}: the points span {extent[0].tolist()} .. {extent[1].tolist()} from origin {list(origin)}, which at an edge of "
                         f"{edge:g} gives indices {min(lo):.0f} .. {max(hi):.0f}; each must be in [0, {CLOUD_INDEX_LIMIT})")


def _cloud_sorted(p, origin, inv):
    n = p.shape[0]
    keys = torch.empty(n, dtype=torch.int64, device=p.device)
    call("mvd_cloud_cell_keys_f32", p.device, p, n, origin[0], origin[1], origin[2], inv, keys)
    return torch.sort(keys, stable=True)


class CloudGrid:
    __slots__ = ("points", "keys", "records", "origin", "cell", "inv")

    def __init__(self, points, keys, records, origin, cell):
        self.points, self.keys, self.records, self.origin, self.cell, self.inv = points, keys, records, origin, cell, 1.0 / cell


@inference_only
def cloud_grid(points, origin, cell, check=True):
    p = _cloud_points(points, "points")
    origin, cell = _cloud_origin(origin), float(cell)
    if not 0.0 < cell < float("inf"):
        raise ValueError(f"cell must be finite and > 0, got {cell}")
    inv = 1.0 / cell
    if check:
        _check_cloud_indices(_cloud_extent(p), origin, inv, "cloud_grid", cell)
    keys, perm = _cloud_sorted(p, origin, inv)
    records = torch.empty((p.shape[0], 4), dtype=torch.float32, device=p.device)
    call("mvd_cloud_grid_build_f32", p.device, p, perm, p.shape[0], records)
    return CloudGrid(p, keys, records, origin, cell)


@inference_only
def cloud_nearest(query, grid, max_dist):
    if not isinstance(grid, CloudGrid):
        raise ValueError(f"grid: expected a CloudGrid (ops.cloud_grid), got {type(grid).__name__}")
    dev = grid.points.device
    max_dist = float(torch.tensor(max_dist, dtype=torch.float32))
    if not 0.0 < max_dist < float("inf"):
        raise ValueError(f"max_dist must be finite and > 0, got {max_dist}")
    if grid.cell < max_dist * CLOUD_CELL_MARGIN * (1 - 1e-12):
        raise ValueError(f"the grid's cell {grid.cell:g} is below max_dist * (1 + 2^-10) = {max_dist * CLOUD_CELL_MARGIN:g}")
    if isinstance(query, CloudGrid):
        if query.origin != grid.origin or query.cell != grid.cell or query.points.device != dev:
            raise ValueError("query and target grids differ in origin, cell or device")
        q = query
    else:
        q = cloud_grid(_cloud_points(query, "query", dev), grid.origin, grid.cell, check=False)
    n, m = q.points.shape[0], grid.points.shape[0]
    dist = torch.empty(n, dtype=torch.float32, device=dev)
    index = torch.empty(n, dtype=torch.int32, device=dev)
    call("mvd_cloud_nearest_f32", dev, q.records, n, grid.records, grid.keys, m, grid.origin[0], grid.origin[1], grid.origin[2], grid.inv,
         max_dist, dist, index)
    return dist, index


@inference_only
def cloud_scores(dist, index, thresholds, points=None, result=None):
    d = L.as_dtype(torch.float32, False, dist, "dist")
    if d.dim() != 1:
        raise ValueError(f"dist must be (n,), got {tuple(d.shape)}")
    n, dev = d.shape[0], d.device
    idx = L.as_dtype(torch.int32, False, index, "index", (n,), dev)
    th = thresholds if isinstance(thresholds, torch.Tensor) else torch.tensor([float(t) for t in thresholds], dtype=torch.float32)
    if th.dim() != 1 or not 1 <= th.shape[0] <= L.MVD_CLOUD_MAX_THRESHOLDS:
        raise ValueError(f"{th.numel()} thresholds, supported 1..{L.MVD_CLOUD_MAX_THRESHOLDS}")
    th = L.as_f32(th.to(dev), "thresholds")
    pts = _cloud_points(points, "points", dev) if points is not None else None
    if pts is not None and pts.shape[0] != n:
        raise ValueError(f"{pts.shape[0]} points for {n} distances")
    if result is None:
        result = torch.empty(10, dtype=torch.int64, device=dev)
    elif result.dtype != torch.int64 or result.device != dev or result.numel() != 10 or not result.is_contiguous():
        raise ValueError("result must be 10 contiguous int64 on dist's device")
    nbytes = L.load().mvd_cloud_scores_workspace_bytes(n)
    ws = workspace(nbytes, dev)
    call("mvd_cloud_scores_f32", dev, d, idx, pts, n, th, th.shape[0], result, ws, int(nbytes))
    return result


def cloud_scores_read(result, T):
    r = result.cpu()
    return float(r[:1].view(torch.float64)[0]), int(r[1]), r[2:2 + T].numpy().copy()


@inference_only
def voxel_downsample(points, voxel, colors=None, origin=None):
    p = _cloud_points(points, "points")
    n, dev = p.shape[0], p.device
    voxel = float(torch.tensor(float(voxel), dtype=torch.float32))
    if not 0.0 < voxel < float("inf"):
        raise ValueError(f"voxel must be finite and > 0, got {voxel}")
    col = None
    if colors is not None:
        col = L.as_f32(colors, "colors", (n, 3), dev)
    inv = 1.0 / voxel
    extent = _cloud_extent(p)
    o = _cloud_origin(origin) if origin is not None else ([0.0, 0.0, 0.0] if extent is None else extent[0].tolist())
    _check_cloud_indices(extent, o, inv, "voxel_downsample", voxel)
    keys, perm = _cloud_sorted(p, o, inv)
    xyz = torch.empty((n, 3), dtype=torch.float32, device=dev)
    rgb = torch.empty((n, 3), dtype=torch.float32, device=dev) if col is not None else None
    counts = torch.empty(n, dtype=torch.int32, device=dev)
    num = torch.empty(1, dtype=torch.int64, device=dev)
    nbytes = L.load().mvd_voxel_reduce_workspace_bytes(n)
    ws = workspace(nbytes, dev)
    call("mvd_voxel_reduce_f32", dev, keys, perm, p, col, n, xyz, rgb, counts, num, ws, int(nbytes))
    k = int(num.item())
    return xyz[:k].clone(), None if rgb is None else rgb[:k].clone(), counts[:k].clone()


class SplitConv2dWeights:
    __slots__ = ("packed", "bias", "cin", "cin_pad", "cout", "kh", "kw", "stride", "mode")

    def __init__(self, packed, bias, cin, cin_pad, cout, kh, kw, stride, mode):
        self.packed, self.bias, self.cin, self.cin_pad, self.cout = packed, bias, cin, cin_pad, cout
        self.kh, self.kw, self.stride, self.mode = kh, kw, stride, mode


@inference_only
def pack_conv2d_weights_split(weight, bias=None, stride=1, mode=L.CONV2D, cin_pad=None):
    wt = L.as_f32(weight, "weight")
    if wt.dim() != 4:
        raise ValueError(f"weight must be 4-D, got {tuple(wt.shape)}")
    if mode == L.DECONV2D:
        cin, cout = wt.shape[0], wt.shape[1]
    else:
        cout, cin = wt.shape[0], wt.shape[1]
    kh, kw = wt.shape[2], wt.shape[3]
    cin_pad = (cin + 7) // 8 * 8 if cin_pad is None else int(cin_pad)
    nbytes = L.load().mvd_conv2d_split_packed_weight_bytes(cin_pad, cout, kh, kw, stride, mode) if cin_pad >= cin else 0
    if nbytes == 0:
        raise ValueError(f"conv2d split: a {kh}x{kw} stride-{stride} layer (mode {mode}) with {cin} (padded {cin_pad}) -> {cout} channels is not built")
    packed = torch.empty(nbytes, dtype=torch.uint8, device=wt.device)
    call("mvd_pack_conv2d_weights_split", wt.device, wt, cin, cin_pad, cout, kh, kw, stride, mode, packed)
    b = None if bias is None else L.as_f32(bias.detach(), "bias", (cout,), wt.device).clone()
    return SplitConv2dWeights(packed, b, cin, cin_pad, cout, kh, kw, stride, mode)


def _nhwc_slice(t, name, channels=None, free_rows=False):
    if not (t.is_cuda and t.dtype == torch.float32 and t.dim() == 4):
        raise ValueError(f"{name} must be a float32 device tensor (B,H,W,C)")
    B, H, W, C = t.shape
    ps = t.stride(2) if W > 1 else max(C, 1)
    rs = t.stride(1) if H > 1 else W * ps
    ims = t.stride(0) if B > 1 else H * rs
    if (C > 1 and t.stride(3) != 1) or ps < C or rs < W * ps or ims < H * rs:
        raise ValueError(f"{name}: a channel slice of a channel-last buffer is needed, got shape {tuple(t.shape)} strides {t.stride()}")
    if not free_rows and (rs != W * ps or ims != H * rs):
        raise ValueError(f"{name}: a channel slice of a DENSE channel-last buffer is needed, got shape {tuple(t.shape)} strides {t.stride()}")
    if channels is not None and C != channels:
        raise ValueError(f"{name}: {C} channels, the layer takes {channels}")
    return B, H, W, C, ps, rs, ims


@inference_only
def conv2d_split(x, x_absmax, wts, act=1, slope=0.2, out=None, out_absmax=None, use_workspace=True, planar_out=False):
    if wts.mode == L.CONV2D_IMAGE:
        xi = L.as_f32(x, "x")
        if xi.dim() != 4 or xi.shape[1] != 3:
            raise ValueError(f"x must be the planar image (B,3,H,W), got {tuple(xi.shape)}")
        B, _, Hi, Wi = xi.shape
        x, xs = xi, 0
    else:
        B, Hi, Wi, _, xs, _, _ = _nhwc_slice(x, "x", wts.cin_pad)
    if wts.mode == L.DECONV2D:
        Ho, Wo = 2 * Hi, 2 * Wi
    else:
        Ho = (Hi + 2 * (wts.kh // 2) - wts.kh) // wts.stride + 1
        Wo = (Wi + 2 * (wts.kw // 2) - wts.kw) // wts.stride + 1
    dev = x.device
    if planar_out:
        if out is not None:
            raise ValueError("planar_out allocates its own output")
        out = torch.empty((B, wts.cout, Ho, Wo), dtype=torch.float32, device=dev)
        ys, rs, ims, cs = 1, Wo, wts.cout * Ho * Wo, Ho * Wo
    else:
        if out is None:
            out = torch.empty((B, Ho, Wo, wts.cout), dtype=torch.float32, device=dev)
        ob, oh, ow, _, ys, rs, ims = _nhwc_slice(out, "out", wts.cout, free_rows=True)
        cs = 1
        if (ob, oh, ow) != (B, Ho, Wo):
            raise ValueError(f"out is {tuple(out.shape)}, the layer writes ({B},{Ho},{Wo},{wts.cout})")
    xam = L.as_f32(x_absmax, "x_absmax", (1,), dev)
    yam = None if out_absmax is None else L.as_f32(out_absmax, "out_absmax", (1,), dev)
    wsb = L.load().mvd_conv2d_split_workspace_bytes(B, Hi, Wi, wts.cin_pad, wts.cout, wts.kh, wts.kw, wts.stride, wts.mode) if use_workspace else 0
    call("mvd_conv2d_split_f32", dev, x, xam, wts.packed, wts.bias, out, yam, B, Hi, Wi, wts.cin_pad, xs, wts.cout, ys, rs, ims, cs,
          wts.kh, wts.kw, wts.stride, wts.mode, int(act), float(slope), workspace(wsb, dev) if wsb else None, wsb)
    return out


@inference_only
def upsample2x_into(x, out, out_absmax=None):
    x = L.as_f32(x, "x")
    B, C, h, w = x.shape
    ob, oh, ow, _, ys, _, _ = _nhwc_slice(out, "out", C)
    if (ob, oh, ow) != (B, 2 * h, 2 * w):
        raise ValueError(f"out is {tuple(out.shape)}, expected ({B},{2 * h},{2 * w},{C})")
    yam = None if out_absmax is None else L.as_f32(out_absmax, "out_absmax", (1,), x.device)
    call("mvd_upsample2x_nhwc_f32", x.device, x, out, yam, B, C, h, w, ys)
    return out


@inference_only
def sweep_corr_nhwc(feat_key, feat_sources, K_key, K_sources, T_src2key, invdepths, corrs, masks, corr_scale=None, corr_absmax=None):
    fk = L.as_f32(feat_key, "feat_key")
    N, h, w, C = fk.shape
    dev = fk.device
    srcs = views(feat_sources, "feat_sources")
    V = len(srcs)
    hs, ws = srcs[0].shape[1] - 3, srcs[0].shape[2] - 3
    srcs = [L.as_f32(s, f"feat_sources[{i}]", (N, hs + 3, ws + 3, C), dev) for i, s in enumerate(srcs)]
    Kk, Ks, Ts, inv, mode = _k1_calibration(K_key, K_sources, T_src2key, invdepths, V, N, h, w, dev)
    S = inv.shape[1]
    if C % 64 != 0:
        raise ValueError(f"feature channels C={C} must be a multiple of 64")
    ps = None
    for name, ts in (("corrs", corrs), ("masks", masks)):
        if len(ts) != V:
            raise ValueError(f"{name}: {len(ts)} entries for {V} views")
        for t in ts:
            b_, h_, w_, _, p_, _, _ = _nhwc_slice(t, name, S)
            if (b_, h_, w_) != (N, h, w) or (ps is not None and p_ != ps):
                raise ValueError(f"{name}: (N,h,w,S) = ({N},{h},{w},{S}) maps with one common pixel stride are needed")
            ps = p_
    cam = None if corr_absmax is None else L.as_f32(corr_absmax, "corr_absmax", (1,), dev)
    call("mvd_sweep_corr_nhwc_f32", dev, fk, srcs, Kk, Ks, Ts, inv, mode, _corr_scale(corr_scale, C), N, C, h, w, hs, ws, S, V,
          list(corrs), list(masks), ps, cam)
    return corrs, masks


@inference_only
def fuse_views_nhwc(corrs, masks, scores, out, out_absmax=None):
    V = len(corrs)
    N, h, w, S, ps, _, _ = _nhwc_slice(corrs[0], "corrs[0]")
    dev = corrs[0].device
    for name, ts in (("corrs", corrs), ("masks", masks)):
        for t in ts:
            if _nhwc_slice(t, name, S)[:5] != (N, h, w, S, ps):
                raise ValueError(f"{name}: equal (N,h,w,S) maps are needed")
    scores = [L.as_f32(s_.reshape(N, h * w), f"scores[{i}]", (N, h * w), dev) for i, s_ in enumerate(views(scores, "scores", V))]
    ob, oh, ow, _, ops_, _, _ = _nhwc_slice(out, "out", S)
    if (ob, oh, ow) != (N, h, w):
        raise ValueError(f"out is {tuple(out.shape)}, expected ({N},{h},{w},{S})")
    yam = None if out_absmax is None else L.as_f32(out_absmax, "out_absmax", (1,), dev)
    call("mvd_fuse_views_nhwc_f32", dev, list(corrs), list(masks), scores, N, S, h, w, V, ps, out, None, ops_, yam)
    return out


@inference_only
def bias_leaky_relu_(x, bias, slope=0.2):
    if not (x.is_cuda and x.dtype == torch.float32 and x.is_contiguous() and x.dim() >= 2):
        raise ValueError("bias_leaky_relu_: x must be a contiguous fp32 device tensor (N,C,...)")
    N, C = x.shape[0], x.shape[1]
    b = L.as_f32(bias, "bias", (C,), x.device)
    call("mvd_bias_leaky_relu_f32", x.device, x, b, N, C, x.numel() // (N * C), float(slope))
    return x


@inference_only
def resize_order1(images, ht, wd):
    x = L.as_f32(images, "images")
    if x.dim() < 2:
        raise ValueError("images must be (..., H, W)")
    hi, wi = x.shape[-2:]
    if ht < hi or wd < wi:
        raise ValueError(f"resize_order1: only upscaling is built ({hi}x{wi} -> {ht}x{wd})")
    planes = x.numel() // (hi * wi)
    y = torch.empty(tuple(x.shape[:-2]) + (ht, wd), dtype=torch.float32, device=x.device)
    call("mvd_resize_order1_f32", x.device, x, y, planes, hi, wi, ht, wd)
    return y


@inference_only
def dispnet_head(x):
    x = L.as_f32(x, "x")
    if x.dim() != 4 or x.shape[1] != 2:
        raise ValueError(f"x must be (N,2,h,w), got {tuple(x.shape)}")
    N, _, h, w = x.shape
    pred = torch.empty_like(x)
    ent = torch.empty((N, 1, h, w), dtype=torch.float32, device=x.device)
    call("mvd_dispnet_head_f32", x.device, x, pred, ent, N, h * w)
    return pred, ent


@inference_only
def to_channels_last_3d(x):
    x = L.as_f32(x, "x")
    B, C, D, h, w = x.shape
    y = torch.empty((B, D, h, w, C), dtype=torch.float32, device=x.device)
    call("mvd_nchw_to_nhwc_f32", x.device, x, y, B, C, D * h * w)
    return y


@inference_only
def from_channels_last_3d(y):
    y = L.as_f32(y, "y")
    B, D, h, w, C = y.shape
    x = torch.empty((B, C, D, h, w), dtype=torch.float32, device=y.device)
    call("mvd_nhwc_to_nchw_f32", y.device, y, x, B, C, D * h * w)
    return x


def _bordered_channels_last(x):
    n, c, h, w = x.shape
    out = torch.zeros((n, h + 3, w + 3, c), dtype=torch.float32, device=x.device)
    out[:, 1:h + 1, 1:w + 1] = x.permute(0, 2, 3, 1)
    return out


def _interior_nchw(g, h, w):
    return g[:, 1:h + 1, 1:w + 1].permute(0, 3, 1, 2).contiguous()


class _WarpVariance(torch.autograd.Function):
    @staticmethod
    def forward(ctx, key_proj_inv, depth_values, n_views, backward, fallback_count, key_feat, *rest):
        srcs, projs = list(rest[:n_views]), list(rest[n_views:])
        ctx.save_for_backward(key_proj_inv, depth_values, key_feat, *srcs, *projs)
        ctx.n_views, ctx.mode, ctx.fallback_count = n_views, backward, fallback_count
        return warp_variance(key_feat.detach(), [s.detach() for s in srcs], projs, key_proj_inv, depth_values)

    @staticmethod
    def backward(ctx, gvar):
        V = ctx.n_views
        kpi, dv, key = ctx.saved_tensors[:3]
        srcs, projs = list(ctx.saved_tensors[3:3 + V]), list(ctx.saved_tensors[3 + V:])
        B, C, h, w = key.shape
        dev = key.device
        with torch.no_grad():
            kb = _bordered_channels_last(key.float())
            sb = [_bordered_channels_last(s.float()) for s in srcs]
            g = gvar.float().permute(0, 2, 3, 4, 1).contiguous()
            gk = torch.empty_like(kb)
            gs = [torch.empty_like(kb) for _ in range(V)]
            projs, kpi, dv = _k3_calibration(projs, kpi, dv, V, B, C, dev)
            if ctx.mode == "gather":
                wsb = L.load().mvd_warp_variance_backward_gather_workspace_bytes(B, C, dv.shape[1], h, w, V)
                call("mvd_warp_variance_backward_gather_f32", dev, kb, sb, projs, kpi, dv, g, B, C, dv.shape[1], h, w, V, gk, gs,
                      ctx.fallback_count, workspace(wsb, dev), wsb)
            else:
                wsb = L.load().mvd_warp_variance_backward_workspace_bytes(B)
                call("mvd_warp_variance_backward_f32", dev, kb, sb, projs, kpi, dv, g, B, C, dv.shape[1], h, w, V, gk, gs,
                      workspace(wsb, dev), wsb)
            out = [None] * 5 + [_interior_nchw(gk, h, w)] + [_interior_nchw(x, h, w) for x in gs] + [None] * V
        return tuple(out)


K3_BACKWARDS = ("atomic", "gather")


def warp_variance_autograd(key_feat, src_feats, src_projs, key_proj_inv, depth_values, backward="atomic", fallback_count=None):
    if backward not in K3_BACKWARDS:
        raise ValueError(f"backward must be 'atomic' or 'gather', got {backward!r}")
    if fallback_count is not None:
        if backward != "gather":
            raise ValueError("fallback_count belongs to backward='gather'")
        if not (isinstance(fallback_count, torch.Tensor) and fallback_count.is_cuda and fallback_count.dtype == torch.int32
                and fallback_count.numel() == 1):
            raise ValueError("fallback_count must be a one-element int32 device tensor")
    srcs = views(src_feats, "src_feats")
    return _WarpVariance.apply(key_proj_inv, depth_values, len(srcs), backward, fallback_count, key_feat, *srcs,
                               *views(src_projs, "src_projs", len(srcs)))


class _SweepCorr(torch.autograd.Function):
    @staticmethod
    def forward(ctx, K_key, invdepths, n_views, corr_scale, feat_key, *rest):
        V = n_views
        srcs, Ks, Ts = list(rest[:V]), list(rest[V:2 * V]), list(rest[2 * V:])
        corrs, masks = sweep_corr(feat_key.detach(), [s.detach() for s in srcs], K_key, Ks, Ts, invdepths, corr_scale)
        ctx.save_for_backward(K_key, invdepths, feat_key, *srcs, *Ks, *Ts)
        ctx.n_views = V
        ctx.corr_scale = corr_scale
        ctx.mark_non_differentiable(*masks)
        return tuple(corrs) + tuple(masks)

    @staticmethod
    def backward(ctx, *grads):
        V = ctx.n_views
        Kk, inv, fk = ctx.saved_tensors[:3]
        srcs = list(ctx.saved_tensors[3:3 + V])
        Ks, Ts = list(ctx.saved_tensors[3 + V:3 + 2 * V]), list(ctx.saved_tensors[3 + 2 * V:])
        N, C, h, w = fk.shape
        hs, ws = srcs[0].shape[-2:]
        S = inv.shape[1]
        dev = fk.device
        with torch.no_grad():
            key = fk.float().permute(0, 2, 3, 1).contiguous()
            sb = [_bordered_channels_last(s.float()) for s in srcs]
            gc = [(g if g is not None else torch.zeros((N, S, h, w), device=dev)).float().contiguous() for g in grads[:V]]
            gk = torch.empty_like(key)
            gs = [torch.empty_like(sb[0]) for _ in range(V)]
            Kk, Ks, Ts, inv, mode = _k1_calibration(Kk, Ks, Ts, inv, V, N, h, w, dev)
            call("mvd_sweep_corr_backward_f32", dev, key, sb, Kk, Ks, Ts, inv, mode, _corr_scale(ctx.corr_scale, C), gc,
                  N, C, h, w, hs, ws, S, V, gk, gs)
            out = [None, None, None, None, gk.permute(0, 3, 1, 2).contiguous()] + [_interior_nchw(x, hs, ws) for x in gs] + [None] * (2 * V)
        return tuple(out)


def sweep_corr_autograd(feat_key, feat_sources, K_key, K_sources, T_src2key, invdepths, corr_scale=None):
    srcs = views(feat_sources, "feat_sources")
    V = len(srcs)
    outs = _SweepCorr.apply(K_key, invdepths, V, corr_scale, feat_key, *srcs, *views(K_sources, "intrinsics_sources", V),
                            *views(T_src2key, "source_to_key_transforms", V))
    return list(outs[:V]), list(outs[V:])


class _SweepWarp(torch.autograd.Function):
    @staticmethod
    def forward(ctx, K_key, invdepths, key_size, n_views, *rest):
        V = n_views
        srcs, Ks, Ts = list(rest[:V]), list(rest[V:2 * V]), list(rest[2 * V:])
        outs, masks = sweep_warp([s.detach() for s in srcs], K_key, Ks, Ts, invdepths, key_size, False)
        ctx.save_for_backward(K_key, invdepths, *Ks, *Ts)
        ctx.n_views, ctx.key_size, ctx.src_shape = V, (int(key_size[0]), int(key_size[1])), tuple(srcs[0].shape)
        ctx.mark_non_differentiable(*masks)
        return tuple(outs) + tuple(masks)

    @staticmethod
    def backward(ctx, *grads):
        V = ctx.n_views
        Kk, inv = ctx.saved_tensors[:2]
        Ks, Ts = list(ctx.saved_tensors[2:2 + V]), list(ctx.saved_tensors[2 + V:])
        N, C, hs, ws = ctx.src_shape
        h, w = ctx.key_size
        dev = Kk.device
        with torch.no_grad():
            Kk, Ks, Ts, inv, mode = _k1_calibration(Kk, Ks, Ts, inv, V, N, h, w, dev)
            S = inv.shape[1]
            gw = [L.as_f32(g, f"grad_warped[{i}]", (N, S, C, h, w), dev) for i, g in enumerate(grads[:V])]
            gs = [torch.empty((N, hs + 3, ws + 3, C), dtype=torch.float32, device=dev) for _ in range(V)]
            call("mvd_sweep_warp_backward_f32", dev, Kk, Ks, Ts, inv, mode, gw, N, C, h, w, hs, ws, S, V, gs)
            gsrc = [_interior_nchw(g, hs, ws) if need else None for g, need in zip(gs, ctx.needs_input_grad[4:4 + V])]
        return (None,) * 4 + tuple(gsrc) + (None,) * (2 * V)


class _ForwardValue(torch.autograd.Function):
    @staticmethod
    def forward(ctx, y, value):
        return value.view_as(y)

    @staticmethod
    def backward(ctx, g):
        return g, None


def sweep_warp_autograd(feat_sources, K_key, K_sources, T_src2key, invdepths, key_size, normalize_after=False):
    srcs = views(feat_sources, "feat_sources")
    V = len(srcs)
    Ks, Ts = views(K_sources, "intrinsics_sources", V), views(T_src2key, "source_to_key_transforms", V)
    outs = _SweepWarp.apply(K_key, invdepths, tuple(key_size), V, *srcs, *Ks, *Ts)
    warped, masks = list(outs[:V]), list(outs[V:])
    if normalize_after:
        exact, _ = sweep_warp([s.detach() for s in srcs], K_key, Ks, Ts, invdepths, key_size, True)
        warped = [_ForwardValue.apply(u / (torch.linalg.norm(u, dim=2, keepdim=True) + 1e-9), e) for u, e in zip(warped, exact)]
    return warped, masks


class _SweepReduce(torch.autograd.Function):
    @staticmethod
    def forward(ctx, depth, mode, groups, pix_offset, stretch, n_views, key_feat, *rest):
        from . import sweep_modes
        V = n_views
        srcs, Ms = list(rest[:V]), list(rest[V:])
        ctx.save_for_backward(depth, key_feat, *srcs, *Ms)
        ctx.cfg = (mode, groups, pix_offset, stretch, V)
        out = sweep_modes.sweep_reduce_inference(key_feat.detach(), [s.detach() for s in srcs], Ms, depth, mode, groups, pix_offset, stretch)
        return tuple(out) if mode == L.REDUCE_GROUPCORR else out

    @staticmethod
    def backward(ctx, *grads):
        from . import sweep_modes
        mode, groups, pix_offset, stretch, V = ctx.cfg
        depth, key = ctx.saved_tensors[:2]
        srcs, Ms = list(ctx.saved_tensors[2:2 + V]), list(ctx.saved_tensors[2 + V:])
        with torch.no_grad():
            kf, srcs, Ms, dv, per_pixel, (B, C, D, h, w, _), (sx, sy) = sweep_modes._reduce_args(key, srcs, Ms, depth, mode, groups, stretch)
            dev = kf.device
            oshape = (B, groups, D, h, w) if mode == L.REDUCE_GROUPCORR else (B, C, D, h, w)
            gout = [L.as_f32(g, f"grad_out[{i}]", oshape, dev) for i, g in enumerate(grads)]
            gk = torch.empty_like(kf)
            gs = [torch.empty_like(kf) for _ in range(V)]
            wsb = L.load().mvd_sweep_reduce_backward_workspace_bytes(B, C, h, w, V)
            call("mvd_sweep_reduce_backward_f32", dev, kf, srcs, Ms, dv, per_pixel, float(pix_offset), float(sx), float(sy), -0.5, mode,
                 groups, gout, B, C, D, h, w, V, gk, gs, workspace(wsb, dev), wsb)
        need = ctx.needs_input_grad
        return (None,) * 6 + (gk if need[6] else None,) + tuple(g if n else None for g, n in zip(gs, need[7:7 + V])) + (None,) * V


def sweep_reduce_autograd(key_feat, src_feats, Ms, depth, mode, groups=1, pix_offset=0.0, stretch=True):
    srcs = views(src_feats, "src_feats")
    out = _SweepReduce.apply(depth, mode, groups, pix_offset, stretch, len(srcs), key_feat, *srcs, *views(Ms, "Ms", len(srcs)))
    return list(out) if mode == L.REDUCE_GROUPCORR else out


class _FuseViews(torch.autograd.Function):
    @staticmethod
    def forward(ctx, n_views, *rest):
        V = n_views
        corrs, masks, scores = list(rest[:V]), list(rest[V:2 * V]), list(rest[2 * V:])
        fused, fmask = fuse_views([c.detach() for c in corrs], [m.detach() for m in masks], [s.detach() for s in scores])
        ctx.save_for_backward(*corrs, *masks, *scores)
        ctx.n_views = V
        ctx.mark_non_differentiable(fmask)
        return fused, fmask

    @staticmethod
    def backward(ctx, gfused, _gmask):
        V = ctx.n_views
        t = ctx.saved_tensors
        corrs, masks, scores = list(t[:V]), list(t[V:2 * V]), list(t[2 * V:])
        N, S, h, w = corrs[0].shape
        dev = corrs[0].device
        with torch.no_grad():
            cs = [L.as_f32(c, f"corrs[{i}]", (N, S, h, w), dev) for i, c in enumerate(corrs)]
            ms = [L.as_f32(m, f"masks[{i}]", (N, S, h, w), dev) for i, m in enumerate(masks)]
            ss = [L.as_f32(s, f"scores[{i}]", (N, 1, h, w), dev) for i, s in enumerate(scores)]
            g = gfused.float().contiguous()
            gcs = [torch.empty_like(cs[0]) for _ in range(V)]
            gss = [torch.empty_like(ss[0]) for _ in range(V)]
            call("mvd_fuse_views_backward_f32", dev, cs, ms, ss, g, N, S, h, w, V, gcs, gss)
        return (None,) + tuple(gcs) + (None,) * V + tuple(gss)


def fuse_views_autograd(corrs, masks, scores):
    corrs = views(corrs, "corrs")
    V = len(corrs)
    return _FuseViews.apply(V, *corrs, *views(masks, "masks", V), *views(scores, "scores", V))


class _SoftmaxRegress(torch.autograd.Function):
    @staticmethod
    def forward(ctx, cost, depth_values):
        c = L.as_f32(cost.detach(), "cost")
        if c.dim() != 4:
            raise ValueError("cost must be (B,D,h,w)")
        B, D, h, w = c.shape
        dv = L.as_f32(depth_values.detach(), "depth_values", (B, D), c.device)
        depth = torch.empty((B, h, w), dtype=torch.float32, device=c.device)
        conf = torch.empty((B, h, w), dtype=torch.float32, device=c.device)
        stats = torch.empty((B, 2, h, w), dtype=torch.float32, device=c.device)
        call("mvd_softmax_regress_stats_f32", c.device, c, dv, B, D, h, w, depth, conf, stats)
        ctx.save_for_backward(c, dv, depth, stats)
        ctx.mark_non_differentiable(conf)
        return depth, conf

    @staticmethod
    def backward(ctx, g_depth, _g_conf):
        c, dv, depth, stats = ctx.saved_tensors
        B, D, h, w = c.shape
        with torch.no_grad():
            g = g_depth.float().contiguous() if g_depth is not None else None
            g_cost = torch.empty_like(c)
            call("mvd_softmax_regress_backward_f32", c.device, c, dv, depth, stats, g, B, D, h, w, g_cost)
        return g_cost, None


def softmax_regress_autograd(cost, depth_values):
    return _SoftmaxRegress.apply(cost, depth_values)


def conv3d_adjoint(weight, mode):
    if weight.dim() != 5 or tuple(weight.shape[2:]) != (3, 3, 3):
        raise ValueError(f"weight must be (*,*,3,3,3), got {tuple(weight.shape)}")
    if mode == L.CONV3D_STRIDE1:
        return weight.flip(2, 3, 4).transpose(0, 1).contiguous(), L.CONV3D_STRIDE1
    if mode == L.CONV3D_STRIDE2:
        return weight, L.DECONV3D_STRIDE2
    if mode == L.DECONV3D_STRIDE2:
        return weight, L.CONV3D_STRIDE2
    raise ValueError(f"mode {mode}")


_IDENTITY_EPILOGUE = {}


def _conv3d_plain(x, weight, mode):
    packed, Cin, Cout = pack_conv3d_weights(weight, mode)
    key = (x.device, Cout)
    if key not in _IDENTITY_EPILOGUE:
        _IDENTITY_EPILOGUE[key] = (torch.ones(Cout, dtype=torch.float32, device=x.device),
                                   torch.zeros(Cout, dtype=torch.float32, device=x.device))
    scale, shift = _IDENTITY_EPILOGUE[key]
    return conv3d_bn_relu(x, packed, Cin, Cout, scale, shift, mode, relu=False)


_MAX_CHAIN = 27 * 8

# ... 70 lines not shown
```

Before: 325.1 depth-maps/sec.

## Add persistent split-fp16 conv kernel with cross-tile prefetch and border-only zeroing

Adds a persistent workgroup variant of the split-fp16 MFMA convolution. Each workgroup loops over tiles and prefetches the next tile's input while computing the current one, with more waves per CU when LDS allows. The channel tile is shrunk for stride-1 3D convs so the grid stays large enough. Separately, the bordered NHWC output buffer is allocated empty and only its pad border is zeroed, instead of zero-filling the whole buffer. The change also factors shared helpers out of the existing kernel and adds experiment env overrides; it costs more code and template instances, and the persistent path's benefit depends on the chosen grid.

```diff
diff --git a/include/mvd.h b/include/mvd.h
--- a/include/mvd.h
+++ b/include/mvd.h
@@ -277,6 +277,8 @@
 int mvd_nchw_to_nhwc_f32(const float* src, float* dst, int N, int C, long long HW, mvd_stream_t stream);
 int mvd_nhwc_to_nchw_f32(const float* src, float* dst, int N, int C, long long HW, mvd_stream_t stream);
 
+int mvd_zero_border_nhwc_f32(float* y, int B, int h, int w, int C, mvd_stream_t stream);
+
 #ifdef __cplusplus
 }
 #endif
diff --git a/robustmvd_amd/_lib.py b/robustmvd_amd/_lib.py
--- a/robustmvd_amd/_lib.py
+++ b/robustmvd_amd/_lib.py
@@ -124,6 +124,7 @@
     "mvd_resize_order1_f32": (_i, [_c_float_p, _c_float_p, ctypes.c_longlong, _i, _i, _i, _i, ctypes.c_void_p]),
     "mvd_nchw_to_nhwc_f32": (_i, [_c_float_p, _c_float_p, _i, _i, ctypes.c_longlong, ctypes.c_void_p]),
     "mvd_nhwc_to_nchw_f32": (_i, [_c_float_p, _c_float_p, _i, _i, ctypes.c_longlong, ctypes.c_void_p]),
+    "mvd_zero_border_nhwc_f32": (_i, [_c_float_p, _i, _i, _i, _i, ctypes.c_void_p]),
     "mvd_depth_eval_workspace_bytes": (_sz, [_i, _i]),
     "mvd_depth_align_stats_f32": (_i, [_c_float_p] * 3 + [ctypes.c_void_p] * 2 + [_i] * 6 + [_c_float_p, ctypes.c_void_p,
                                                                                             ctypes.c_void_p, _sz, ctypes.c_void_p]),
diff --git a/robustmvd_amd/blocks.py b/robustmvd_amd/blocks.py
--- a/robustmvd_amd/blocks.py
+++ b/robustmvd_amd/blocks.py
@@ -215,8 +215,10 @@
         return pk
 
     @ops.inference_only
-    def forward_layout(self, x, out_layout, return_absmax=False):
+    def forward_layout(self, x, out_layout, return_absmax=False, out=None):
         pk = self._prepare()
+        if out is not None and not (self.split_layers and out_layout == L.LAYOUT_NHWC_BORDER):
+            raise ValueError("out: only the split layers' LAYOUT_NHWC_BORDER output can be written into a caller's buffer")
         if not self.split_layers:
             for i, (w, cin, cout, k, stride, scale, shift, relu) in enumerate(pk.layers):
                 x = ops.conv2d_bn_relu(x, w, cin, cout, k, stride, scale, shift, relu=relu,
@@ -240,7 +242,11 @@
                     slots[7:8] = ops.absmax(x)
             elif out_layout == L.LAYOUT_NHWC_BORDER:
                 B, h, w_, _ = x.shape
-                buf = torch.zeros((B, h + 3, w_ + 3, wts.cout), dtype=torch.float32, device=x.device)
+                if out is None:
+                    out = torch.empty((B, h + 3, w_ + 3, wts.cout), dtype=torch.float32, device=x.device)
+                elif tuple(out.shape) != (B, h + 3, w_ + 3, wts.cout):
+                    raise ValueError(f"out: shape {tuple(out.shape)}, expected {(B, h + 3, w_ + 3, wts.cout)}")
+                buf = ops.zero_border_nhwc(out)
                 ops.conv2d_split(x, a_in, wts, act=0, out=buf[:, 1:h + 1, 1:w_ + 1, :], out_absmax=slots[7:8])
                 x = buf
             else:
diff --git a/robustmvd_amd/csrc/conv2d_split.hip b/robustmvd_amd/csrc/conv2d_split.hip
--- a/robustmvd_amd/csrc/conv2d_split.hip
+++ b/robustmvd_amd/csrc/conv2d_split.hip
@@ -61,6 +61,7 @@
     int pad_y, pad_x;
     int Cout, ncp;
     int tiles_x, tiles_y, nblocks, ksplit, chunks_per_split;
+    int tiles;
     int ncls;
     long long cls_bytes;
     int act;
@@ -171,6 +172,88 @@
     }
 }
 
+struct C2Tile {
+    int nb, ks, cls, b, od, bb, oy0, ox0, iy0, ix0;
+};
+template <int S>
+__device__ __forceinline__ C2Tile c2_tile(const C2Params& p, int bx) {
+    C2Tile t;
+    t.nb = bx % p.nblocks; bx /= p.nblocks;
+    t.ks = bx % p.ksplit; bx /= p.ksplit;
+    t.cls = bx % p.ncls; bx /= p.ncls;
+    const int tx = bx % p.tiles_x; bx /= p.tiles_x;
+    const int ty = bx % p.tiles_y;
+    t.b = bx / p.tiles_y;
+    t.od = t.b % p.Do; t.bb = t.b / p.Do;
+    t.oy0 = ty * C2_TH; t.ox0 = tx * C2_TW;
+    t.iy0 = t.oy0 * S - (p.pad_y - (t.cls >> 1)); t.ix0 = t.ox0 * S - (p.pad_x - (t.cls & 1));
+    return t;
+}
+__device__ __forceinline__ void c2_xscale(const float* xamax, float& xsc, float& xsc_inv) {
+    const unsigned mb = __builtin_amdgcn_readfirstlane((int)__float_as_uint(*xamax));
+    const int ex = (int)((mb >> 23) & 0xffu) - 127;
+    const int e = max(-125, min(125, ex - 14));
+    xsc = __uint_as_float((unsigned)(127 - e) << 23);
+    xsc_inv = __uint_as_float((unsigned)(127 + e) << 23);
+}
+__device__ __forceinline__ void c2_split2(float xsc, float a0, float a1, unsigned& hi, unsigned& lo) {
+    const float one = 1.0f;
+    unsigned hp, lp;
+    float t0, t1;
+    asm("v_fma_mixlo_f16 %0, %1, %2, 0 op_sel:[0,0,0] op_sel_hi:[0,0,0]" : "=v"(hp) : "v"(a0), "s"(xsc));
+    asm("v_fma_mixhi_f16 %0, %1, %2, 0 op_sel:[0,0,0] op_sel_hi:[0,0,0]" : "+v"(hp) : "v"(a1), "s"(xsc));
+    asm("v_fma_mix_f32 %0, %1, %2, -%3 op_sel:[0,0,0] op_sel_hi:[0,0,1]" : "=v"(t0) : "v"(a0), "s"(xsc), "v"(hp));
+    asm("v_fma_mix_f32 %0, %1, %2, -%3 op_sel:[0,0,1] op_sel_hi:[0,0,1]" : "=v"(t1) : "v"(a1), "s"(xsc), "v"(hp));
+    asm("v_fma_mixlo_f16 %0, %1, %2, 0 op_sel:[0,0,0] op_sel_hi:[0,0,0]" : "=v"(lp) : "v"(t0), "s"(one));
+    asm("v_fma_mixhi_f16 %0, %1, %2, 0 op_sel:[0,0,0] op_sel_hi:[0,0,0]" : "+v"(lp) : "v"(t1), "s"(one));
+    hi = hp;
+    lo = lp;
+}
+template <class G, int KW, int S, int U8, int STEPS, bool NCHW3>
+__device__ __forceinline__ void c2_tapoff(int (&tapoff)[STEPS], int g, int px16, int row0) {
+#pragma unroll
+    for (int s = 0; s < STEPS; ++s) {
+        if constexpr (NCHW3) {
+            tapoff[s] = (s * G::PW + 2 * px16 + 2 * g) * G::PB + row0 * G::ROWB;
+        } else {
+            int unit = 4 * s + g;
+            if (unit >= G::UNITS) unit = 0;
+            const int tap = unit / U8, c8 = unit % U8, ky = tap / KW, kx = tap % KW;
+            tapoff[s] = ((ky * S + kx % S) * G::PWS + kx / S + px16) * G::PB + c8 * G::C8S + row0 * G::ROWB;
+        }
+    }
+}
+template <class G, int MTW, int NTW>
+__device__ __forceinline__ void c2_kstep(const char* a, const c2h8 (&wh)[NTW], const c2h8 (&wl)[NTW], c2f4 (&acc)[MTW][NTW]) {
+    constexpr int PLANE = G::PLANE;
+    c2h8 xh = *reinterpret_cast<const c2h8*>(a), xl = *reinterpret_cast<const c2h8*>(a + PLANE);
+    c2h8 yh = xh, yl = xl;
+    if (MTW > 1) {
+        yh = *reinterpret_cast<const c2h8*>(a + G::ROWB);
+        yl = *reinterpret_cast<const c2h8*>(a + G::ROWB + PLANE);
+    }
+#pragma unroll
+    for (int m = 0; m < MTW; ++m) {
+        const c2h8 ch = xh, cl = xl;
+        xh = yh; xl = yl;
+        if (m + 2 < MTW && !(C2_KO & 8)) {
+            yh = *reinterpret_cast<const c2h8*>(a + (m + 2) * G::ROWB);
+            yl = *reinterpret_cast<const c2h8*>(a + (m + 2) * G::ROWB + PLANE);
+        }
+#pragma unroll
+        for (int t = 0; t < NTW; ++t) {
+            if (C2_KO & 2) {
+                acc[m][t][0] += (float)ch[0] * (float)wh[t][0] + (float)cl[1] * (float)wl[t][1];
+                continue;
+            }
+            acc[m][t] = __builtin_amdgcn_mfma_f32_16x16x32_f16(wh[t], ch, acc[m][t], 0, 0, 0);
+            acc[m][t] = __builtin_amdgcn_mfma_f32_16x16x32_f16(wl[t], ch, acc[m][t], 0, 0, 0);
+            acc[m][t] = __builtin_amdgcn_mfma_f32_16x16x32_f16(wh[t], cl, acc[m][t], 0, 0, 0);
+        }
+        __builtin_amdgcn_sched_barrier(0);
+    }
+}
+
 template <int KH, int KW, int S, int U8, int WM, int NTW, bool NCHW3>
 __global__ void __launch_bounds__(256, 2) conv2d_split_kernel(C2Params p) {
     const float amax_seen = absmax_seen(p.part ? nullptr : p.yamax);
@@ -182,39 +265,13 @@
     const int wm = wv / WN, wn = wv % WN;
     const int g = lane >> 4, px16 = lane & 15;
 
-    int bx = blockIdx.x;
-    const int nb = bx % p.nblocks; bx /= p.nblocks;
-    const int ks = bx % p.ksplit; bx /= p.ksplit;
-    const int cls = bx % p.ncls; bx /= p.ncls;
-    const int tx = bx % p.tiles_x; bx /= p.tiles_x;
-    const int ty = bx % p.tiles_y;
-    const int b = bx / p.tiles_y;
-    const int od = b % p.Do, bb = b / p.Do;
-    const int ca = cls >> 1, cb2 = cls & 1;
-    const int oy0 = ty * C2_TH, ox0 = tx * C2_TW;
-    const int iy0 = oy0 * S - (p.pad_y - ca), ix0 = ox0 * S - (p.pad_x - cb2);
+    const C2Tile tl = c2_tile<S>(p, blockIdx.x);
+    const int nb = tl.nb, ks = tl.ks, cls = tl.cls, b = tl.b, od = tl.od, bb = tl.bb;
+    const int oy0 = tl.oy0, ox0 = tl.ox0, iy0 = tl.iy0, ix0 = tl.ix0;
 
     float xsc, xsc_inv;
-    {
-        const unsigned mb = __builtin_amdgcn_readfirstlane((int)__float_as_uint(*p.xamax));
-        const int ex = (int)((mb >> 23) & 0xffu) - 127;
-        const int e = max(-125, min(125, ex - 14));
-        xsc = __uint_as_float((unsigned)(127 - e) << 23);
-        xsc_inv = __uint_as_float((unsigned)(127 + e) << 23);
-    }
-    const float one = 1.0f;
-    auto split2 = [xsc, one](float a0, float a1, unsigned& hi, unsigned& lo) {
-        unsigned hp, lp;
-        float t0, t1;
-        asm("v_fma_mixlo_f16 %0, %1, %2, 0 op_sel:[0,0,0] op_sel_hi:[0,0,0]" : "=v"(hp) : "v"(a0), "s"(xsc));
-        asm("v_fma_mixhi_f16 %0, %1, %2, 0 op_sel:[0,0,0] op_sel_hi:[0,0,0]" : "+v"(hp) : "v"(a1), "s"(xsc));
-        asm("v_fma_mix_f32 %0, %1, %2, -%3 op_sel:[0,0,0] op_sel_hi:[0,0,1]" : "=v"(t0) : "v"(a0), "s"(xsc), "v"(hp));
-        asm("v_fma_mix_f32 %0, %1, %2, -%3 op_sel:[0,0,1] op_sel_hi:[0,0,1]" : "=v"(t1) : "v"(a1), "s"(xsc), "v"(hp));
-        asm("v_fma_mixlo_f16 %0, %1, %2, 0 op_sel:[0,0,0] op_sel_hi:[0,0,0]" : "=v"(lp) : "v"(t0), "s"(one));
-        asm("v_fma_mixhi_f16 %0, %1, %2, 0 op_sel:[0,0,0] op_sel_hi:[0,0,0]" : "+v"(lp) : "v"(t1), "s"(one));
-        hi = hp;
-        lo = lp;
-    };
+    c2_xscale(p.xamax, xsc, xsc_inv);
+    auto split2 = [xsc](float a0, float a1, unsigned& hi, unsigned& lo) { c2_split2(xsc, a0, a1, hi, lo); };
 
     long long goff[G::NIT];
     int loff[G::NIT];
@@ -235,17 +292,7 @@
         }
     }
     int tapoff[STEPS];
-#pragma unroll
-    for (int s = 0; s < STEPS; ++s) {
-        if constexpr (NCHW3) {
-            tapoff[s] = (s * G::PW + 2 * px16 + 2 * g) * PB + wm * MTW * G::ROWB;
-        } else {
-            int unit = 4 * s + g;
-            if (unit >= G::UNITS) unit = 0;
-            const int tap = unit / U8, c8 = unit % U8, ky = tap / KW, kx = tap % KW;
-            tapoff[s] = ((ky * S + kx % S) * G::PWS + kx / S + px16) * PB + c8 * G::C8S + wm * MTW * G::ROWB;
-        }
-    }
+    c2_tapoff<G, KW, S, U8, STEPS, NCHW3>(tapoff, g, px16, wm * MTW);
 
     const int nt0 = nb * (WN * NTW) + wn * NTW;
     const size_t nt_stride = (size_t)p.nchunks * STEPS * 2048;
@@ -326,33 +373,7 @@
                 }
                 wc += 2048;
             }
-            const char* a = patch + tapoff[s];
-            c2h8 xh = *reinterpret_cast<const c2h8*>(a), xl = *reinterpret_cast<const c2h8*>(a + PLANE);
-            c2h8 yh = xh, yl = xl;
-            if (MTW > 1) {
-                yh = *reinterpret_cast<const c2h8*>(a + G::ROWB);
-                yl = *reinterpret_cast<const c2h8*>(a + G::ROWB + PLANE);
-            }
-#pragma unroll
-            for (int m = 0; m < MTW; ++m) {
-                const c2h8 ch = xh, cl = xl;
-                xh = yh; xl = yl;
-                if (m + 2 < MTW && !(C2_KO & 8)) {
-                    yh = *reinterpret_cast<const c2h8*>(a + (m + 2) * G::ROWB);
-                    yl = *reinterpret_cast<const c2h8*>(a + (m + 2) * G::ROWB + PLANE);
-                }
-#pragma unroll
-                for (int t = 0; t < NTW; ++t) {
-                    if (C2_KO & 2) {
-                        acc[m][t][0] += (float)ch[0] * (float)wh[t][0] + (float)cl[1] * (float)wl[t][1];
-                        continue;
-                    }
-                    acc[m][t] = __builtin_amdgcn_mfma_f32_16x16x32_f16(wh[t], ch, acc[m][t], 0, 0, 0);
-                    acc[m][t] = __builtin_amdgcn_mfma_f32_16x16x32_f16(wl[t], ch, acc[m][t], 0, 0, 0);
-                    acc[m][t] = __builtin_amdgcn_mfma_f32_16x16x32_f16(wh[t], cl, acc[m][t], 0, 0, 0);
-                }
-                __builtin_amdgcn_sched_barrier(0);
-            }
+            c2_kstep<G, MTW, NTW>(patch + tapoff[s], wh, wl, acc);
 #pragma unroll
             for (int t = 0; t < NTW; ++t) { wh[t] = nh[t]; wl[t] = nl[t]; }
         }
@@ -384,6 +405,137 @@
         }
     }
     if (p.yamax && !p.part) {
+        for (int o = 32; o > 0; o >>= 1) amax = fmaxf(amax, __shfl_xor(amax, o));
+        if (lane == 0) wmax[wv] = amax;
+        __syncthreads();
+        if (tid == 0) {
+            amax = fmaxf(fmaxf(wmax[0], wmax[1]), fmaxf(wmax[2], wmax[3]));
+            raise_absmax_seen(p.yamax, amax, amax_seen);
+        }
+    }
+}
+
+template <int KH, int KW, int S, int U8, int WM, int NTW, int WAVES>
+__global__ void __launch_bounds__(256, WAVES) conv2d_split_persist_kernel(C2Params p) {
+    const float amax_seen = absmax_seen(p.yamax);
+    using G = C2Geom<KH, KW, S, U8, false>;
+    constexpr int WN = 4 / WM, MTW = 16 / WM, STEPS = G::STEPS, PB = G::PB, PLANE = G::PLANE;
+    extern __shared__ __attribute__((aligned(16))) char patch[];
+    float* const wmax = reinterpret_cast<float*>(patch + 2 * PLANE);
+    const int tid = threadIdx.x, lane = tid & 63, wv = tid >> 6;
+    const int wm = wv / WN, wn = wv % WN;
+    const int g = lane >> 4, px16 = lane & 15;
+    int t = blockIdx.x;
+    if (t >= p.tiles) return;
+
+    float xsc, xsc_inv;
+    c2_xscale(p.xamax, xsc, xsc_inv);
+    int loff[G::NIT];
+#pragma unroll
+    for (int k = 0; k < G::NIT; ++k) {
+        const int it = tid + 256 * k, pix = it / U8, c8 = it % U8, py = pix / G::PW, pxx = pix % G::PW;
+        loff[k] = it < G::ITEMS ? ((py * S + pxx % S) * G::PWS + pxx / S) * PB + c8 * G::C8S : -1;
+    }
+    int tapoff[STEPS];
+    c2_tapoff<G, KW, S, U8, STEPS, false>(tapoff, g, px16, wm * MTW);
+    const size_t nt_stride = (size_t)p.nchunks * STEPS * 2048;
+    const size_t plane_floats = (size_t)p.Hi * p.Wi * p.xs;
+
+    int goff[G::NIT];
+    c2f4 v0[G::NIT], v1[G::NIT];
+    bool zlive;
+    auto prefetch = [&](const C2Tile& tl, int chunk, bool new_tile) {
+        if (new_tile) {
+#pragma unroll
+            for (int k = 0; k < G::NIT; ++k) {
+                const int it = tid + 256 * k, pix = it / U8, c8 = it % U8, py = pix / G::PW, pxx = pix % G::PW;
+                const int iy = tl.iy0 + py, ix = tl.ix0 + pxx;
+                const bool inside = it < G::ITEMS && iy >= 0 && iy < p.Hi && ix >= 0 && ix < p.Wi;
+                goff[k] = inside ? (iy * p.Wi + ix) * p.xs + c8 * 8 : -1;
+            }
+        }
+        const int kd = chunk / p.nchunks_c, zi = tl.od * p.SD - p.pad_d + kd;
+        zlive = zi >= 0 && zi < p.Di;
+        const float* xim = p.x + ((size_t)tl.bb * p.Di + (zlive ? zi : 0)) * plane_floats + (size_t)(chunk - kd * p.nchunks_c) * G::CC;
+#pragma unroll
+        for (int k = 0; k < G::NIT; ++k) {
+            const float* a = xim + max(goff[k], 0);
+            v0[k] = *reinterpret_cast<const c2f4*>(a);
+            v1[k] = *reinterpret_cast<const c2f4*>(a + 4);
+        }
+    };
+
+    C2Tile tl = c2_tile<S>(p, t);
+    prefetch(tl, 0, true);
+    C2Chan kc[NTW];
+    int nb_have = -1;
+    float amax = 0.f;
+    for (;;) {
+        const int nt0 = tl.nb * (WN * NTW) + wn * NTW;
+        const char* const wlane = p.wpk + (size_t)tl.cls * p.cls_bytes + (size_t)nt0 * nt_stride + lane * 16;
+        if (tl.nb != nb_have) {
+#pragma unroll
+            for (int q = 0; q < NTW; ++q) kc[q] = c2_chan(p, (nt0 + q) * 16 + 4 * g, xsc_inv);
+            nb_have = tl.nb;
+        }
+        const int tn = t + (int)gridDim.x;
+        const bool more = tn < p.tiles;
+        const C2Tile tnext = c2_tile<S>(p, more ? tn : t);
+
+        c2f4 acc[MTW][NTW];
+#pragma unroll
+        for (int m = 0; m < MTW; ++m)
+#pragma unroll
+            for (int q = 0; q < NTW; ++q) acc[m][q] = c2f4{0, 0, 0, 0};
+
+        for (int chunk = 0; chunk < p.nchunks; ++chunk) {
+            c2h8 wh[STEPS][NTW], wl[STEPS][NTW];
+            const char* const wc = wlane + (size_t)chunk * STEPS * 2048;
+#pragma unroll
+            for (int s = 0; s < STEPS; ++s)
+#pragma unroll
+                for (int q = 0; q < NTW; ++q) {
+                    wh[s][q] = *reinterpret_cast<const c2h8*>(wc + s * 2048 + q * nt_stride);
+                    wl[s][q] = *reinterpret_cast<const c2h8*>(wc + s * 2048 + q * nt_stride + 1024);
+                }
+            __builtin_amdgcn_sched_barrier(0);
+            __syncthreads();
+#pragma unroll
+            for (int k = 0; k < G::NIT; ++k) {
+                if (loff[k] < 0) continue;
+                if (goff[k] < 0 || !zlive) v0[k] = v1[k] = c2f4{0, 0, 0, 0};
+                unsigned h0, h1, h2, h3, l0, l1, l2, l3;
+                c2_split2(xsc, v0[k][0], v0[k][1], h0, l0);
+                c2_split2(xsc, v0[k][2], v0[k][3], h1, l1);
+                c2_split2(xsc, v1[k][0], v1[k][1], h2, l2);
+                c2_split2(xsc, v1[k][2], v1[k][3], h3, l3);
+                *reinterpret_cast<c2u4*>(patch + loff[k]) = c2u4{h0, h1, h2, h3};
+                *reinterpret_cast<c2u4*>(patch + loff[k] + PLANE) = c2u4{l0, l1, l2, l3};
+            }
+            __builtin_amdgcn_sched_barrier(0);
+            const bool last = chunk + 1 == p.nchunks;
+            prefetch(last ? tnext : tl, last ? 0 : chunk + 1, last);
+            __builtin_amdgcn_sched_barrier(0);
+            __syncthreads();
+#pragma unroll
+            for (int s = 0; s < STEPS; ++s) c2_kstep<G, MTW, NTW>(patch + tapoff[s], wh[s], wl[s], acc);
+        }
+
+        const int ox = tl.ox0 + px16;
+#pragma unroll
+        for (int q = 0; q < NTW; ++q) {
+            const int cb = (nt0 + q) * 16 + 4 * g;
+            if (cb >= p.Cout || ox >= p.Wo) continue;
+            const size_t o0 = c2_out_offset(p, tl.bb, tl.od, tl.oy0 + wm * MTW, ox, tl.cls, cb), ostep = c2_row_step(p);
+#pragma unroll
+            for (int m = 0; m < MTW; ++m)
+                if (tl.oy0 + wm * MTW + m < p.Ho) c2_finish(p, o0 + m * ostep, cb, acc[m][q], kc[q], amax);
+        }
+        if (!more) break;
+        t = tn;
+        tl = tnext;
+    }
+    if (p.yamax) {
         for (int o = 32; o > 0; o >>= 1) amax = fmaxf(amax, __shfl_xor(amax, o));
         if (lane == 0) wmax[wv] = amax;
         __syncthreads();
@@ -575,9 +727,37 @@
 struct C2Plan {
     int Ho, Wo, tiles_x, tiles_y, bn, nblocks, ncp, ncls, nchunks, ksplit;
     long long tiles;
+    long long persist;
     size_t part_bytes;
 };
-static C2Plan c2_plan(const C2Shape& s, int B, int Hi, int Wi, int cin_pad, int cout, int KH, int KW, int stride) {
+
+enum { C2_K33 = 0, C2_K33W = 1, C2_K33S2 = 2, C2_K55S2 = 3, C2_NOT_PERSISTENT = -1 };
+static int c2_persist_kind(const C2Shape& s) {
+    if (s.nchw3 || s.transposed) return C2_NOT_PERSISTENT;
+    if (s.KH == 3 && s.KW == 3 && s.S == 1) return s.U8 == 4 ? C2_K33W : s.U8 == 1 ? C2_K33 : C2_NOT_PERSISTENT;
+    if (s.KH == 3 && s.KW == 3 && s.S == 2 && s.U8 == 1) return C2_K33S2;
+    if (s.KH == 5 && s.KW == 5 && s.S == 2 && s.U8 == 1) return C2_K55S2;
+    return C2_NOT_PERSISTENT;
+}
+constexpr int C2_PERSIST_WGS[4][3] = {
+    {4, 0, 0},
+    {0, 0, 0},
+    {0, 0, 0},
+    {0, 0, 0},
+};
+static long long c2_persist_grid(const C2Shape& s, const C2Plan& q, int Hi, int Wi, int xs) {
+    const int kind = c2_persist_kind(s);
+    if (kind == C2_NOT_PERSISTENT || q.bn > 64 || q.ksplit != 1 || q.tiles > 0x7fffffffLL || (long long)Hi * Wi * xs > 0x7fffffffLL) return 0;
+    const int wgs = C2_PERSIST_WGS[kind][q.bn == 16 ? 0 : q.bn == 32 ? 1 : 2];
+    if (const char* e = exp_env("MVD_C2_PERSIST")) {
+        const long long v = atoll(e);
+        if (v <= 0) return 0;
+        if (v > 1) return std::min<long long>(v, q.tiles);
+    }
+    if (wgs == 0) return 0;
+    return std::min(q.tiles, (256LL * wgs + q.nblocks - 1) / q.nblocks * q.nblocks);
+}
+static C2Plan c2_plan(const C2Shape& s, int B, int Hi, int Wi, int cin_pad, int xs, int cout, int KH, int KW, int stride) {
     C2Plan q{};
     if (s.transposed) { q.Ho = Hi; q.Wo = Wi; q.ncls = 4; }
     else { q.Ho = (Hi + 2 * (KH / 2) - KH) / stride + 1; q.Wo = (Wi + 2 * (KW / 2) - KW) / stride + 1; q.ncls = 1; }
@@ -596,6 +776,7 @@
         if (v >= 1 && v <= 32 && (v & (v - 1)) == 0 && v <= q.nchunks) q.ksplit = v;
     }
     q.part_bytes = q.ksplit > 1 ? (size_t)q.ksplit * q.ncls * B * q.Ho * q.Wo * q.ncp * sizeof(float) : 0;
+    q.persist = c2_persist_grid(s, q, Hi, Wi, xs);
     return q;
 }
 
@@ -610,6 +791,16 @@
     hipLaunchKernelGGL(kern, dim3((unsigned)nblk), dim3(256), lds, st, p);
     return launch_status("conv2d_split");
 }
+template <int KH, int KW, int S, int U8, int WM>
+static int c2_launch_persist(const C2Params& p, long long grid, hipStream_t st) {
+    using G = C2Geom<KH, KW, S, U8, false>;
+    constexpr int WAVES = (G::STEPS == 3 && (G::NIT <= 2 || WM == 4)) ? 3 : 2;
+    auto kern = conv2d_split_persist_kernel<KH, KW, S, U8, WM, 1, WAVES>;
+    constexpr int lds = 2 * G::PLANE + 16;
+    static_assert(lds <= 48 * 1024, "the persistent form: three workgroups per CU, no LDS attribute");
+    hipLaunchKernelGGL(kern, dim3((unsigned)grid), dim3(256), lds, st, p);
+    return launch_status("conv2d_split: persistent");
+}
 
 template <int KH, int KW, int S, int U8, bool NCHW3>
 static int c2_launch_bn(const C2Params& p, int bn, long long nblk, hipStream_t st) {
@@ -621,8 +812,31 @@
     }
     return MVD_ERR_INVALID_ARG;
 }
-
-static int c2_dispatch(const C2Shape& s, const C2Params& p, int bn, long long nblk, hipStream_t st) {
+template <int KH, int KW, int S, int U8>
+static int c2_launch_persist_bn(const C2Params& p, int bn, long long grid, hipStream_t st) {
+    switch (bn) {
+#ifdef MVD_EXPERIMENTS
+        case 64: return c2_launch_persist<KH, KW, S, U8, 1>(p, grid, st);
+        case 32: return c2_launch_persist<KH, KW, S, U8, 2>(p, grid, st);
+#endif
+        case 16: return c2_launch_persist<KH, KW, S, U8, 4>(p, grid, st);
+    }
+    return MVD_ERR_INVALID_ARG;
+}
+
+static int c2_dispatch(const C2Shape& s, C2Params& p, int bn, long long nblk, long long persist, hipStream_t st) {
+    if (persist > 0 && p.ksplit == 1) {
+        p.tiles = (int)nblk;
+        switch (c2_persist_kind(s)) {
+            case C2_K33: return c2_launch_persist_bn<3, 3, 1, 1>(p, bn, persist, st);
+#ifdef MVD_EXPERIMENTS
+            case C2_K33W: return c2_launch_persist_bn<3, 3, 1, 4>(p, bn, persist, st);
+            case C2_K33S2: return c2_launch_persist_bn<3, 3, 2, 1>(p, bn, persist, st);
+            case C2_K55S2: return c2_launch_persist_bn<5, 5, 2, 1>(p, bn, persist, st);
+#endif
+        }
+        return MVD_ERR_INVALID_ARG;
+    }
     if (s.nchw3) return c2_launch_bn<7, 7, 2, 1, true>(p, bn, nblk, st);
     if (s.KH == 1) return c2_launch_bn<1, 1, 1, 4, false>(p, bn, nblk, st);
     if (s.KH == 2) return s.U8 == 4 ? c2_launch_bn<2, 2, 1, 4, false>(p, bn, nblk, st) : c2_launch_bn<2, 2, 1, 2, false>(p, bn, nblk, st);
@@ -663,7 +877,7 @@
 size_t mvd_conv2d_split_workspace_bytes(int B, int Hi, int Wi, int Cin_pad, int Cout, int KH, int KW, int stride, int mode) {
     mvd::C2Shape s;
     if (B <= 0 || Hi <= 0 || Wi <= 0 || Cin_pad <= 0 || Cout <= 0 || !mvd::c2_shape(KH, KW, stride, mode, Cin_pad, &s)) return 0;
-    return mvd::c2_plan(s, B, Hi, Wi, Cin_pad, Cout, KH, KW, stride).part_bytes;
+    return mvd::c2_plan(s, B, Hi, Wi, Cin_pad, Cin_pad, Cout, KH, KW, stride).part_bytes;
 }
 
 int mvd_conv2d_split_f32(const float* x, const float* x_absmax, const void* packed_w, const float* bias, float* y, float* y_absmax, int B,
@@ -690,7 +904,7 @@
     p.Cout = Cout; p.ys = y_pixel_stride; p.act = act; p.slope = slope;
     const size_t fb = mvd::c2_frag_bytes(s, Cin_pad, Cout);
     p.eun = reinterpret_cast<const float*>(static_cast<const char*>(packed_w) + fb);
-    const mvd::C2Plan q = mvd::c2_plan(s, B, Hi, Wi, Cin_pad, Cout, KH, KW, stride);
+    const mvd::C2Plan q = mvd::c2_plan(s, B, Hi, Wi, Cin_pad, x_pixel_stride, Cout, KH, KW, stride);
     p.Ho = q.Ho; p.Wo = q.Wo; p.ncls = q.ncls;
     if (s.transposed) {
         p.Hy = 2 * Hi; p.Wy = 2 * Wi; p.oy_mul = p.ox_mul = 2; p.pad_y = p.pad_x = 1;
@@ -716,7 +930,7 @@
     p.part = ksplit > 1 ? static_cast<float*>(workspace) : nullptr;
     const long long nblk = tiles * ksplit;
     MVD_REQUIRE(nblk <= 0x7fffffffLL, "conv2d_split: %lld workgroups exceed the grid limit", nblk);
-    int rc = mvd::c2_dispatch(s, p, bn, nblk, st);
+    int rc = mvd::c2_dispatch(s, p, bn, nblk, q.persist, st);
     if (rc != MVD_OK || ksplit == 1) return rc;
     const long long n = (long long)B * p.Ho * p.Wo * ((Cout + 3) / 4);
     MVD_REQUIRE(n < 0x7fffffffLL, "conv2d_split: split reduction over %lld outputs", n);
@@ -789,14 +1003,22 @@
     q.tiles_y = (q.Ho + mvd::C2_TH - 1) / mvd::C2_TH;
     q.tiles_x = (q.Wo + mvd::C2_TW - 1) / mvd::C2_TW;
     q.bn = mvd::c2_bn(ncout);
+    const long long planes = (long long)q.tiles_x * q.tiles_y * B * *Do;
+    if (mode == MVD_CONV3D_STRIDE1 && !mvd::exp_env("MVD_C2_BN") && planes * ((ncout + q.bn - 1) / q.bn) >= 128)
+        while (q.bn > 16 && planes * ((ncout + q.bn - 1) / q.bn) < 512) q.bn /= 2;
     q.nblocks = (ncout + q.bn - 1) / q.bn;
     q.ncp = q.nblocks * q.bn;
     q.nchunks = (mode == MVD_DECONV3D_STRIDE2 ? 2 : 3) * (Cin / (8 * s.U8));
-    q.tiles = (long long)q.tiles_x * q.tiles_y * B * *Do * q.nblocks;
+    q.tiles = planes * q.nblocks;
     q.ksplit = 1;
     if (q.tiles < 128)
         while (q.tiles * q.ksplit < 320 && q.ksplit < 32 && q.nchunks / (q.ksplit * 2) >= 2) q.ksplit *= 2;
+    if (const char* e = mvd::exp_env("MVD_C2_KSPLIT")) {
+        const int v = atoi(e);
+        if (v >= 1 && v <= 32 && (v & (v - 1)) == 0 && v <= q.nchunks) q.ksplit = v;
+    }
     q.part_bytes = q.ksplit > 1 ? (size_t)q.ksplit * B * *Do * q.Ho * q.Wo * q.ncp * sizeof(float) : 0;
+    q.persist = mvd::c2_persist_grid(s, q, Hi, Wi, Cin);
     return q;
 }
 
@@ -841,7 +1063,9 @@
     p.part = ksplit > 1 ? static_cast<float*>(workspace) : nullptr;
     const long long nblk = q.tiles * ksplit;
     MVD_REQUIRE(nblk <= 0x7fffffffLL, "conv3d_igemm: %lld workgroups exceed the grid limit", nblk);
-    int rc = mvd::c2_dispatch(s, p, q.bn, nblk, st);
+    MVD_REQUIRE(q.nblocks * (q.bn / 16) <= mvd::c2_ntiles(ncout), "conv3d_igemm: channel tile %d reads past the %d packed fragments", q.bn,
+                mvd::c2_ntiles(ncout));
+    int rc = mvd::c2_dispatch(s, p, q.bn, nblk, q.persist, st);
     if (rc != MVD_OK || ksplit == 1) return rc;
     const long long n = (long long)p.B * p.Ho * p.Wo * ((p.Cout + 3) / 4);
     MVD_REQUIRE(n < 0x7fffffffLL, "conv3d_igemm: split reduction over %lld outputs", n);
diff --git a/robustmvd_amd/csrc/resize.hip b/robustmvd_amd/csrc/resize.hip
--- a/robustmvd_amd/csrc/resize.hip
+++ b/robustmvd_amd/csrc/resize.hip
@@ -44,6 +44,35 @@
     dst[(plane * ho + y) * (size_t)wo + x] = (float)t;
 }
 
+__global__ void __launch_bounds__(256) zero_border_nhwc_kernel(float* __restrict__ y, int h, int w, int c4n, int n) {
+    const int i = blockIdx.x * 256 + threadIdx.x;
+    if (i >= n) return;
+    const int c4 = i % c4n, bp = i / c4n, wp = w + 3;
+    int row, col;
+    if (bp < 3 * wp) {
+        const int r = bp / wp;
+        row = r == 0 ? 0 : h + r;
+        col = bp - r * wp;
+    } else {
+        const int q = bp - 3 * wp, r = q / 3, k = q - 3 * r;
+        row = 1 + r;
+        col = k == 0 ? 0 : w + k;
+    }
+    float* o = y + (((size_t)blockIdx.y * (h + 3) + row) * wp + col) * (4 * (size_t)c4n) + 4 * c4;
+    *reinterpret_cast<float4*>(o) = float4{0.f, 0.f, 0.f, 0.f};
+}
+
+}
+
+extern "C" int mvd_zero_border_nhwc_f32(float* y, int B, int h, int w, int C, mvd_stream_t stream) {
+    MVD_REQUIRE(y, "zero_border_nhwc: NULL argument");
+    MVD_REQUIRE(B > 0 && B <= 65535 && h > 0 && w > 0 && C > 0 && C % 4 == 0, "zero_border_nhwc: bad dimensions (C a multiple of 4, B 1..65535)");
+    MVD_REQUIRE(((uintptr_t)y & 15) == 0, "zero_border_nhwc: y must be 16-byte aligned");
+    const long long n = (3LL * (w + 3) + 3LL * h) * (C / 4);
+    MVD_REQUIRE(n < 0x7fffffffLL, "zero_border_nhwc: %lld border items", n);
+    hipLaunchKernelGGL(mvd::zero_border_nhwc_kernel, dim3((unsigned)((n + 255) / 256), (unsigned)B), dim3(256), 0, (hipStream_t)stream, y, h, w,
+                       C / 4, (int)n);
+    return mvd::launch_status("zero_border_nhwc");
 }
 
 extern "C" int mvd_resize_order1_f32(const float* src, float* dst, long long planes, int hi, int wi, int ho, int wo,
diff --git a/robustmvd_amd/ops.py b/robustmvd_amd/ops.py
--- a/robustmvd_amd/ops.py
+++ b/robustmvd_amd/ops.py
@@ -946,6 +946,17 @@
 
 
 @inference_only
+def zero_border_nhwc(buf):
+    if not (isinstance(buf, torch.Tensor) and buf.is_cuda and buf.dtype == torch.float32 and buf.is_contiguous() and buf.dim() == 4):
+        raise ValueError("zero_border_nhwc: buf must be a contiguous (B, h + 3, w + 3, C) fp32 device tensor")
+    B, hp, wp, C = buf.shape
+    if hp < 4 or wp < 4 or C % 4:
+        raise ValueError(f"zero_border_nhwc: shape {tuple(buf.shape)} (h, w >= 1, C a multiple of 4)")
+    call("mvd_zero_border_nhwc_f32", buf.device, buf, B, hp - 3, wp - 3, C)
+    return buf
+
+
+@inference_only
 def to_channels_last_3d(x):
     x = L.as_f32(x, "x")
     B, C, D, h, w = x.shape
```

Measured after the change: 333.5 depth-maps/sec (median of 6 runs). 2.6% higher.
